# mKaloer/TFServingCache

Hardware: AMD Instinct MI355X
Metric: predict req/sec (whole node) (higher is better)
Workload: dtype bf16; 1 GPU; model=resnet50_v1.5, global_batch=8, seq_len=224, parallelism=ring-sharded serving x1, mode=headline (lru), full=False, batch_per_request=8, threads=10, n_models=1000, model_repo=hardlinked copies of one SavedModel per family (content-dedup applies), provider=disk, pool_size=10, n_cold_loads=1030, transport=real gRPC (native nghttp2 front-end) over TCP loopback, client_channels=1, hipgraph=True

## Files before the change

tfservingcache_amd/engine/csrc/executor.cpp:

```cpp
#include <torch/extension.h>

#include <hip/hip_runtime.h>

#include <c10/hip/HIPStream.h>

#include <cstdint>
#include <stdexcept>
#include <vector>

#include "kernels.h"

namespace tfsc {

enum CallKind : int {
  K_ELT_UNARY = 0,
  K_ELT_BINARY,
  K_BN_ACT,
  K_SOFTMAX,
  K_LAYERNORM,
  K_MEAN_LAST,
  K_MEAN_MID,
  K_POOL,
  K_TRANSPOSE,
  K_GATHER,
  K_PAD_NHWC,
  K_GEMM,
  K_BGEMM,
  K_IM2COL,
  K_CONV,
  K_PAD_LAST,
  K_ATTENTION,
  K_DEPTHWISE,
  K_GEMM_FP8,
  K_QUANT_FP8,
  K_CAST,
  K_ARGMAX_LAST,
  K_SCATTER,
  K_RESIZE,
  K_ZERO_INSERT,
};

struct Call {
  int kind;
  std::vector<intptr_t> ptrs;
  std::vector<int64_t> ints;
  std::vector<float> floats;
};

static void launch_call(const Call& c, hipStream_t s) {
  auto p = [&](int i) { return reinterpret_cast<ushort*>(c.ptrs[i]); };
  auto cp = [&](int i) { return reinterpret_cast<const ushort*>(c.ptrs[i]); };
  const auto& I = c.ints;
  switch (c.kind) {
    case K_ELT_UNARY:
      launch_eltwise_unary(s, cp(0), p(1), I[0], int(I[1]));
      break;
    case K_ELT_BINARY: {
      BcastArgs bc;
      bc.ndim = int(I[2]);
      for (int d = 0; d < MAX_DIMS; ++d) {
        bc.dims[d] = d < bc.ndim ? I[3 + d] : 1;
        bc.sa[d] = d < bc.ndim ? I[3 + bc.ndim + d] : 0;
        bc.sb[d] = d < bc.ndim ? I[3 + 2 * bc.ndim + d] : 0;
      }
      launch_eltwise_binary(s, cp(0), cp(1), p(2), I[0], bc, int(I[1]));
      break;
    }
    case K_BN_ACT:
      launch_bn_act(s, cp(0), cp(1), cp(2), p(3), I[0], I[1], int(I[2]));
      break;
    case K_SOFTMAX:
      launch_softmax(s, cp(0), p(1), I[0], I[1]);
      break;
    case K_LAYERNORM:
      launch_layernorm(s, cp(0), cp(1), cp(2), p(3), I[0], I[1],
                       c.floats[0]);
      break;
    case K_MEAN_LAST:
      launch_reduce_mean_last(s, cp(0), p(1), I[0], I[1]);
      break;
    case K_MEAN_MID:
      launch_reduce_mean_mid(s, cp(0), p(1), I[0], I[1], I[2]);
      break;
    case K_POOL:
      launch_pool(s, cp(0), p(1), I[0] != 0, int(I[1]), int(I[2]),
                  int(I[3]), int(I[4]), int(I[5]), int(I[6]), int(I[7]),
                  int(I[8]), int(I[9]), int(I[10]), int(I[11]), int(I[12]));
      break;
    case K_TRANSPOSE: {
      int ndim = int(I[0]);
      launch_transpose(s, cp(0), p(1), ndim, I.data() + 1,
                       I.data() + 1 + ndim, I[1 + 2 * ndim]);
      break;
    }
    case K_GATHER:
      launch_gather_rows(s, cp(0), reinterpret_cast<const int*>(c.ptrs[1]),
                         p(2), I[0], I[1]);
      break;
    case K_PAD_NHWC:
      launch_pad_nhwc(s, cp(0), p(1), int(I[0]), int(I[1]), int(I[2]),
                      int(I[3]), int(I[4]), int(I[5]), int(I[6]),
                      int(I[7]));
      break;
    case K_GEMM: {
      const ushort* bias = c.ptrs[2] ? cp(2) : nullptr;
      const ushort* res = c.ptrs[3] ? cp(3) : nullptr;
      launch_gemm(s, cp(0), cp(1), bias, res, p(4), I[0], I[1], I[2],
                  int(I[3]), c.floats[0]);
      break;
    }
    case K_BGEMM:
      launch_batched_gemm(s, cp(0), cp(1), p(2), I[0], I[1], I[2], I[3],
                          I[4], I[5], I[6], I[7] != 0, c.floats[0]);
      break;
    case K_IM2COL:
      launch_im2col(s, cp(0), p(1), int(I[0]), int(I[1]), int(I[2]),
                    int(I[3]), int(I[4]), int(I[5]), int(I[6]), int(I[7]),
                    int(I[8]), int(I[9]), int(I[10]), int(I[11]),
                    int(I[12]));
      break;
    case K_CONV: {
      const ushort* res = c.ptrs[3] ? cp(3) : nullptr;
      launch_conv_igemm(s, cp(0), cp(1), cp(2), res, cp(4), p(5),
                        int(I[0]), int(I[1]), int(I[2]), int(I[3]),
                        int(I[4]), int(I[5]), int(I[6]), int(I[7]),
                        int(I[8]), int(I[9]), int(I[10]), int(I[11]),
                        int(I[12]), int(I[13]), int(I[14]));
      break;
    }
    case K_PAD_LAST:
      launch_pad_last(s, cp(0), p(1), I[0], int(I[1]), int(I[2]));
      break;
    case K_ATTENTION: {
      const ushort* abias =
          c.ptrs.size() > 4 && c.ptrs[4] ? cp(4) : nullptr;
      if (abias && I.size() < 7)
        throw std::runtime_error("attention bias needs [sb, sh, sq]");
      launch_attention(s, cp(0), cp(1), cp(2), p(3), int(I[0]), int(I[1]),
                       int(I[2]), int(I[3]), c.floats[0], abias,
                       abias ? I[4] : 0, abias ? I[5] : 0,
                       abias ? I[6] : 0);
      break;
    }
    case K_GEMM_FP8: {
      const ushort* bias8 = c.ptrs[4] ? cp(4) : nullptr;
      const ushort* res8 = c.ptrs[5] ? cp(5) : nullptr;
      launch_gemm_fp8(s, reinterpret_cast<const uint8_t*>(c.ptrs[0]),
                      reinterpret_cast<const float*>(c.ptrs[1]),
                      reinterpret_cast<const uint8_t*>(c.ptrs[2]),
                      reinterpret_cast<const float*>(c.ptrs[3]),
                      bias8, res8, p(6), I[0], I[1], I[2], int(I[3]));
      break;
    }
    case K_QUANT_FP8:
      launch_quant_rowwise(s, cp(0),
                           reinterpret_cast<uint8_t*>(c.ptrs[1]),
                           reinterpret_cast<float*>(c.ptrs[2]),
                           I[0], I[1], I[2]);
      break;
    case K_SCATTER: {
      int nd = int(I[0]);
      launch_scatter(s, cp(0), p(1), nd, I.data() + 1, I.data() + 1 + nd,
                     I[1 + 2 * nd]);
      break;
    }
    case K_CAST:
      launch_cast(s, reinterpret_cast<const void*>(c.ptrs[0]),
                  reinterpret_cast<void*>(c.ptrs[1]), I[0], int(I[1]));
      break;
    case K_ARGMAX_LAST:
      launch_argmax_last(s, cp(0), reinterpret_cast<int*>(c.ptrs[1]),
                         I[0], I[1]);
      break;
    case K_DEPTHWISE:
      launch_depthwise_conv(s, cp(0), cp(1), cp(2), p(3), int(I[0]),
                            int(I[1]), int(I[2]), int(I[3]), int(I[4]),
                            int(I[5]), int(I[6]), int(I[7]), int(I[8]),
                            int(I[9]), int(I[10]), int(I[11]),
                            int(I[12]));
      break;
    case K_RESIZE: {
      if (c.ptrs.size() != 2 || I.size() != 9)
        throw std::runtime_error("resize needs 2 ptrs and 9 ints");
      for (int k = 0; k < 7; ++k)
        if (I[k] < 0 || I[k] > INT32_MAX)
          throw std::runtime_error("resize: int out of range");
      launch_resize_nhwc(s, cp(0), p(1), int(I[0]), int(I[1]), int(I[2]),
                         int(I[3]), int(I[4]), int(I[5]), int(I[6]),
                         I[7] != 0, I[8] != 0);
      break;
    }
    case K_ZERO_INSERT: {
      if (c.ptrs.size() != 2 || I.size() != 6)
        throw std::runtime_error("zero_insert needs 2 ptrs and 6 ints");
      for (int k = 0; k < 6; ++k)
        if (I[k] < 0 || I[k] > INT32_MAX)
          throw std::runtime_error("zero_insert: int out of range");
      launch_zero_insert_nhwc(s, cp(0), p(1), int(I[0]), int(I[1]),
                              int(I[2]), int(I[3]), int(I[4]), int(I[5]));
      break;
    }
    default:
      throw std::runtime_error("unknown call kind " +
                               std::to_string(c.kind));
  }
}

class ExecPlan {
 public:
  explicit ExecPlan(const std::vector<Call>& calls) : calls_(calls) {}

  void run() {
    hipStream_t s = c10::hip::getCurrentHIPStream().stream();
    for (const auto& c : calls_) launch_call(c, s);
    hipError_t e = hipGetLastError();
    if (e != hipSuccess)
      throw std::runtime_error(std::string("kernel launch failed: ") +
                               hipGetErrorString(e));
  }

  void capture() {
    hipStream_t s = c10::hip::getCurrentHIPStream().stream();
    if (graph_exec_) return;
    hipGraph_t graph = nullptr;
    if (hipStreamBeginCapture(s, hipStreamCaptureModeThreadLocal) !=
        hipSuccess)
      throw std::runtime_error("hipStreamBeginCapture failed");
    for (const auto& c : calls_) launch_call(c, s);
    if (hipStreamEndCapture(s, &graph) != hipSuccess)
      throw std::runtime_error("hipStreamEndCapture failed");
    hipGraphExec_t ge = nullptr;
    if (hipGraphInstantiate(&ge, graph, nullptr, nullptr, 0) != hipSuccess) {
      hipGraphDestroy(graph);
      throw std::runtime_error("hipGraphInstantiate failed");
    }
    hipGraphDestroy(graph);
    graph_exec_ = ge;
  }

  bool has_graph() const { return graph_exec_ != nullptr; }

  void run_graph() {
    if (!graph_exec_) {
      run();
      return;
    }
    hipStream_t s = c10::hip::getCurrentHIPStream().stream();
    if (hipGraphLaunch(graph_exec_, s) != hipSuccess)
      throw std::runtime_error("hipGraphLaunch failed");
  }

  ~ExecPlan() {
    if (graph_exec_) hipGraphExecDestroy(graph_exec_);
  }

  void run_on(hipStream_t s) {
    if (graph_exec_) {
      if (hipGraphLaunch(graph_exec_, s) != hipSuccess)
        throw std::runtime_error("hipGraphLaunch failed");
      return;
    }
    for (const auto& c : calls_) launch_call(c, s);
    hipError_t e = hipGetLastError();
    if (e != hipSuccess)
      throw std::runtime_error(std::string("kernel launch failed: ") +
                               hipGetErrorString(e));
  }

  size_t n_calls() const { return calls_.size(); }

 private:
  std::vector<Call> calls_;
  hipGraphExec_t graph_exec_ = nullptr;
};

void fast_run_plan(void* plan, hipStream_t s) {
  reinterpret_cast<ExecPlan*>(plan)->run_on(s);
}

struct PtrDesc {
  uint8_t tag;
  int32_t reg = 0;
  int64_t off = 0;
};

class CallTemplate {
 public:
  std::vector<Call> calls;
  std::vector<std::vector<PtrDesc>> descs;

  ExecPlan* instantiate(uintptr_t ws,
                        const std::vector<uintptr_t>& bases) const {
    std::vector<Call> out = calls;
    for (size_t i = 0; i < out.size(); ++i) {
      auto& ds = descs[i];
      auto& ptrs = out[i].ptrs;
      ptrs.resize(ds.size());
      for (size_t j = 0; j < ds.size(); ++j) {
        const PtrDesc& d = ds[j];
        if (d.tag == 0)
          ptrs[j] = intptr_t(ws) + d.off;
        else if (d.tag == 1)
          ptrs[j] = intptr_t(bases.at(size_t(d.reg))) + d.off;
        else
          ptrs[j] = 0;
      }
    }
    return new ExecPlan(out);
  }
};

}

namespace py = pybind11;

void register_fastpath(py::module_& mod);
void register_frontend(py::module_& mod);
void register_rest_frontend(py::module_& mod);

PYBIND11_MODULE(TORCH_EXTENSION_NAME, mod) {
  using tfsc::Call;
  using tfsc::ExecPlan;

  py::class_<ExecPlan>(mod, "ExecPlan")
      .def(py::init([](py::list calls) {
        std::vector<Call> cs;
        cs.reserve(calls.size());
        for (auto item : calls) {
          py::tuple t = item.cast<py::tuple>();
          Call c;
          c.kind = t[0].cast<int>();
          c.ptrs = t[1].cast<std::vector<intptr_t>>();
          c.ints = t[2].cast<std::vector<int64_t>>();
          c.floats = t[3].cast<std::vector<float>>();
          cs.push_back(std::move(c));
        }
        return new ExecPlan(cs);
      }))
      .def("run", &ExecPlan::run, py::call_guard<py::gil_scoped_release>())
      .def("capture", &ExecPlan::capture,
           py::call_guard<py::gil_scoped_release>())
      .def("run_graph", &ExecPlan::run_graph,
           py::call_guard<py::gil_scoped_release>())
      .def("has_graph", &ExecPlan::has_graph)
      .def("n_calls", &ExecPlan::n_calls)
      .def("ptr", [](ExecPlan& p) {
        return reinterpret_cast<uintptr_t>(&p);
      });

  mod.attr("K_ELT_UNARY") = int(tfsc::K_ELT_UNARY);
  mod.attr("K_ELT_BINARY") = int(tfsc::K_ELT_BINARY);
  mod.attr("K_BN_ACT") = int(tfsc::K_BN_ACT);
  mod.attr("K_SOFTMAX") = int(tfsc::K_SOFTMAX);
  mod.attr("K_LAYERNORM") = int(tfsc::K_LAYERNORM);
  mod.attr("K_MEAN_LAST") = int(tfsc::K_MEAN_LAST);
  mod.attr("K_MEAN_MID") = int(tfsc::K_MEAN_MID);
  mod.attr("K_POOL") = int(tfsc::K_POOL);
  mod.attr("K_TRANSPOSE") = int(tfsc::K_TRANSPOSE);
  mod.attr("K_GATHER") = int(tfsc::K_GATHER);
  mod.attr("K_PAD_NHWC") = int(tfsc::K_PAD_NHWC);
  mod.attr("K_GEMM") = int(tfsc::K_GEMM);
  mod.attr("K_BGEMM") = int(tfsc::K_BGEMM);
  mod.attr("K_IM2COL") = int(tfsc::K_IM2COL);
  mod.attr("K_CONV") = int(tfsc::K_CONV);
  mod.attr("K_PAD_LAST") = int(tfsc::K_PAD_LAST);
  mod.attr("K_ATTENTION") = int(tfsc::K_ATTENTION);
  mod.attr("K_DEPTHWISE") = int(tfsc::K_DEPTHWISE);
  mod.attr("K_GEMM_FP8") = int(tfsc::K_GEMM_FP8);
  mod.attr("K_QUANT_FP8") = int(tfsc::K_QUANT_FP8);
  mod.attr("K_CAST") = int(tfsc::K_CAST);
  mod.attr("K_ARGMAX_LAST") = int(tfsc::K_ARGMAX_LAST);
  mod.attr("K_SCATTER") = int(tfsc::K_SCATTER);
  mod.attr("K_RESIZE") = int(tfsc::K_RESIZE);
  mod.attr("K_ZERO_INSERT") = int(tfsc::K_ZERO_INSERT);

  py::class_<tfsc::CallTemplate>(mod, "CallTemplate")
      .def(py::init([](py::list calls) {
        auto* t = new tfsc::CallTemplate();
        t->calls.reserve(calls.size());
        t->descs.reserve(calls.size());
        for (auto item : calls) {
          py::tuple tu = item.cast<py::tuple>();
          Call c;
          c.kind = tu[0].cast<int>();
          std::vector<tfsc::PtrDesc> ds;
          for (auto dd : tu[1].cast<py::list>()) {
            py::tuple dt = dd.cast<py::tuple>();
            tfsc::PtrDesc d;
            d.tag = uint8_t(dt[0].cast<int>());
            if (d.tag == 0) {
              d.off = dt[1].cast<int64_t>();
            } else if (d.tag == 1) {
              d.reg = dt[1].cast<int32_t>();
              d.off = dt[2].cast<int64_t>();
            }
            ds.push_back(d);
          }
          c.ints = tu[2].cast<std::vector<int64_t>>();
          c.floats = tu[3].cast<std::vector<float>>();
          t->calls.push_back(std::move(c));
          t->descs.push_back(std::move(ds));
        }
        return t;
      }));

  mod.def("instantiate_plan",
          [](const tfsc::CallTemplate& t, uintptr_t ws,
             const std::vector<uintptr_t>& bases) {
            return std::unique_ptr<ExecPlan>(t.instantiate(ws, bases));
          });

  register_fastpath(mod);
  register_frontend(mod);
  register_rest_frontend(mod);

  mod.attr("ELT_ADD") = int(tfsc::ELT_ADD);
  mod.attr("ELT_SUB") = int(tfsc::ELT_SUB);
  mod.attr("ELT_MUL") = int(tfsc::ELT_MUL);
  mod.attr("ELT_DIV") = int(tfsc::ELT_DIV);
  mod.attr("ELT_MAX") = int(tfsc::ELT_MAX);
  mod.attr("ELT_MIN") = int(tfsc::ELT_MIN);
  mod.attr("ELT_SQDIFF") = int(tfsc::ELT_SQDIFF);
  mod.attr("ELT_RELU") = int(tfsc::ELT_RELU);
  mod.attr("ELT_TANH") = int(tfsc::ELT_TANH);
  mod.attr("ELT_SIGMOID") = int(tfsc::ELT_SIGMOID);
  mod.attr("ELT_ERF") = int(tfsc::ELT_ERF);
  mod.attr("ELT_SQRT") = int(tfsc::ELT_SQRT);
  mod.attr("ELT_RSQRT") = int(tfsc::ELT_RSQRT);
  mod.attr("ELT_EXP") = int(tfsc::ELT_EXP);
  mod.attr("ELT_NEG") = int(tfsc::ELT_NEG);
  mod.attr("ELT_SQUARE") = int(tfsc::ELT_SQUARE);
  mod.attr("ELT_GELU") = int(tfsc::ELT_GELU);
  mod.attr("ELT_RELU6") = int(tfsc::ELT_RELU6);

  mod.attr("ACT_NONE") = int(tfsc::ACT_NONE);
  mod.attr("ACT_RELU") = int(tfsc::ACT_RELU);
  mod.attr("ACT_TANH") = int(tfsc::ACT_TANH);
  mod.attr("ACT_SIGMOID") = int(tfsc::ACT_SIGMOID);
  mod.attr("ACT_GELU") = int(tfsc::ACT_GELU);
  mod.attr("ACT_RELU6") = int(tfsc::ACT_RELU6);
}
```

tfservingcache_amd/engine/csrc/ops/attention.hip:

```cpp
#include "../common.h"
#include "../kernels.h"

#include <climits>
#include <stdexcept>

namespace tfsc {

namespace attn {

using bf16x8_t = __attribute__((ext_vector_type(8))) __bf16;
using f32x4_t = __attribute__((ext_vector_type(4))) float;
using ushort2_t = __attribute__((ext_vector_type(2))) ushort;

constexpr int D = 64;
constexpr int QBLK = 64;
constexpr int KVBLK = 64;
constexpr int NW = 4;
constexpr int THREADS = NW * WAVE;

TFSC_DEV int t_off(int row, int chunk) {
  return row * 128 + ((chunk ^ (row & 7)) << 4);
}

TFSC_DEV int p_off(int row, int chunk) {
  return row * 256 + ((chunk ^ (row & 7)) << 4);
}

TFSC_DEV void stage_rows_glds(const ushort* __restrict__ src, int64_t ld,
                              int row0, int row_limit, char* lds_tile,
                              int wave, int lane) {
  int r_in = lane >> 3, chunk = lane & 7;
  #pragma unroll
  for (int i = 0; i < 2; ++i) {
    int row = wave * 16 + i * 8 + r_in;
    int grow = row0 + row;
    grow = grow < row_limit ? grow : row_limit;
    int chunk_src = chunk ^ (row & 7);
    const ushort* gptr = src + (int64_t)grow * ld + chunk_src * 8;
    char* lds_base = lds_tile + (wave * 16 + i * 8) * 128;
    __builtin_amdgcn_global_load_lds(
        reinterpret_cast<const uint32_t*>(gptr),
        reinterpret_cast<uint32_t*>(lds_base), 16, 0, 0);
  }
}

TFSC_DEV void stage_vt(const ushort* __restrict__ src, int64_t ld,
                       int row0, int row_limit, ushort* lds_tile,
                       int wave, int lane) {
  int tid = wave * WAVE + lane;
  #pragma unroll
  for (int pass = 0; pass < 2; ++pass) {
    int idx = pass * THREADS + tid;
    int kv = idx >> 3;
    int dg = idx & 7;
    int gkv = row0 + kv;
    gkv = gkv < row_limit ? gkv : row_limit;
    const ushort* gptr = src + (int64_t)gkv * ld + dg * 8;
    short8_t v = *reinterpret_cast<const short8_t*>(gptr);
    #pragma unroll
    for (int j = 0; j < 8; ++j) {
      int d = dg * 8 + j;
      int byte_off = t_off(d, kv >> 3) + (kv & 7) * 2;
      *reinterpret_cast<ushort*>(
          reinterpret_cast<char*>(lds_tile) + byte_off) = ushort(v[j]);
    }
  }
}

template <int RING, bool HAS_BIAS>
__global__ __launch_bounds__(THREADS)
void attention_kernel(const ushort* __restrict__ Q,
                      const ushort* __restrict__ K,
                      const ushort* __restrict__ V,
                      ushort* __restrict__ O,
                      int B, int S, int H, float scale, int n_qblk,
                      const ushort* __restrict__ bias, int64_t bias_sb,
                      int64_t bias_sh, int bias_sq) {
  __shared__ __attribute__((aligned(16))) char smem[8192 * (2 * RING + 2)];
  auto k_lds = [&](int buf) -> char* { return smem + buf * 8192; };
  auto vt_lds = [&](int buf) -> char* {
    return smem + RING * 8192 + buf * 8192;
  };
  char* q_lds = smem + 2 * RING * 8192;
  char* p_lds = smem + 2 * RING * 8192;

  const int flat = blockIdx.x;
  const int qb = flat % n_qblk;
  const int h = (flat / n_qblk) % H;
  const int b = flat / (n_qblk * H);
  const int64_t ld = (int64_t)H * D;
  const ushort* Qb = Q + (int64_t)b * S * ld + h * D;
  const ushort* Kb = K + (int64_t)b * S * ld + h * D;
  const ushort* Vb = V + (int64_t)b * S * ld + h * D;
  ushort* Ob = O + (int64_t)b * S * ld + h * D;

  const int wave = threadIdx.x / WAVE;
  const int lane = threadIdx.x % WAVE;
  const int frow = lane & 15;
  const int kgrp = lane >> 4;
  const int q0 = qb * QBLK;

  stage_rows_glds(Qb, ld, q0, S - 1, q_lds, wave, lane);
  stage_rows_glds(Kb, ld, 0, S - 1, k_lds(0), wave, lane);
  stage_vt(Vb, ld, 0, S - 1, reinterpret_cast<ushort*>(vt_lds(0)), wave,
           lane);
  stage_rows_glds(Kb, ld, KVBLK, S - 1, k_lds(1), wave, lane);
  stage_vt(Vb, ld, KVBLK, S - 1, reinterpret_cast<ushort*>(vt_lds(1)),
           wave, lane);
  __syncthreads();
  bf16x8_t qf[2];
  #pragma unroll
  for (int ks = 0; ks < 2; ++ks) {
    int row = wave * 16 + frow;
    qf[ks] = *reinterpret_cast<const bf16x8_t*>(
        q_lds + t_off(row, ks * 4 + kgrp));
  }
  __syncthreads();

  float m_run[4], l_run[4];
  f32x4_t o_acc[4] = {};
  #pragma unroll
  for (int r = 0; r < 4; ++r) {
    m_run[r] = HAS_BIAS ? -1.0e38f : -3.0e38f;
    l_run[r] = 0.f;
  }

  const char* bias_bh = nullptr;
  uint32_t bias_roff[4] = {};
  if (HAS_BIAS) {
    bias_bh = reinterpret_cast<const char*>(
        bias + (int64_t)b * bias_sb + (int64_t)h * bias_sh);
    #pragma unroll
    for (int r = 0; r < 4; ++r) {
      int qrow = q0 + wave * 16 + kgrp * 4 + r;
      qrow = qrow < S ? qrow : S - 1;
      bias_roff[r] = uint32_t(qrow) * uint32_t(bias_sq) * 2u;
    }
  }

  const int n_kv = (S + KVBLK - 1) / KVBLK;
  const int n_pair = (n_kv + 1) / 2;

  for (int t = 0; t < n_pair; ++t) {
    if (t > 0) __syncthreads();
    const int base = RING >= 4 ? (t & 1) * 2 : 0;
    const int kv_base = t * 2 * KVBLK;
    ushort2_t bv[4][4] = {};
    if (HAS_BIAS) {
      uint32_t off[8];
      #pragma unroll
      for (int ni = 0; ni < 8; ++ni) {
        int kv_col = kv_base + ni * 16 + frow;
        off[ni] = uint32_t(kv_col < S ? kv_col : S - 1) * 2u;
      }
      if (bias_sq == 0) {
        ushort bk[8];
        #pragma unroll
        for (int ni = 0; ni < 8; ++ni)
          bk[ni] = *reinterpret_cast<const ushort*>(bias_bh + off[ni]);
        #pragma unroll
        for (int ni = 0; ni < 8; ++ni)
          #pragma unroll
          for (int r = 0; r < 4; ++r) bv[ni & 3][r][ni >> 2] = bk[ni];
      } else {
        #pragma unroll
        for (int ni = 0; ni < 8; ++ni)
          #pragma unroll
          for (int r = 0; r < 4; ++r)
            bv[ni & 3][r][ni >> 2] = *reinterpret_cast<const ushort*>(
                bias_bh + (bias_roff[r] + off[ni]));
      }
    }
    if (RING >= 4 && t + 1 < n_pair) {
      const int nb = ((t + 1) & 1) * 2;
      stage_rows_glds(Kb, ld, (2 * t + 2) * KVBLK, S - 1, k_lds(nb),
                      wave, lane);
      stage_vt(Vb, ld, (2 * t + 2) * KVBLK, S - 1,
               reinterpret_cast<ushort*>(vt_lds(nb)), wave, lane);
      stage_rows_glds(Kb, ld, (2 * t + 3) * KVBLK, S - 1, k_lds(nb + 1),
                      wave, lane);
      stage_vt(Vb, ld, (2 * t + 3) * KVBLK, S - 1,
               reinterpret_cast<ushort*>(vt_lds(nb + 1)), wave, lane);
    }

    f32x4_t sc[8] = {};
    #pragma unroll
    for (int half = 0; half < 2; ++half) {
      const char* kt = k_lds(base + half);
      #pragma unroll
      for (int ks = 0; ks < 2; ++ks) {
        #pragma unroll
        for (int ni = 0; ni < 4; ++ni) {
          bf16x8_t kf = *reinterpret_cast<const bf16x8_t*>(
              kt + t_off(ni * 16 + frow, ks * 4 + kgrp));
          sc[half * 4 + ni] = __builtin_amdgcn_mfma_f32_16x16x32_bf16(
              qf[ks], kf, sc[half * 4 + ni], 0, 0, 0);
        }
      }
    }
    #pragma unroll
    for (int ni = 0; ni < 8; ++ni) {
      int kv_col = kv_base + ni * 16 + frow;
      bool valid = kv_col < S;
      #pragma unroll
      for (int r = 0; r < 4; ++r) {
        float v = sc[ni][r] * scale;
        if (HAS_BIAS) v += bf2f(bv[ni & 3][r][ni >> 2]);
        sc[ni][r] = valid ? v : -3.0e38f;
      }
    }

    float pmax[4];
    #pragma unroll
    for (int r = 0; r < 4; ++r) {
      float v = sc[0][r];
      #pragma unroll
      for (int ni = 1; ni < 8; ++ni) v = fmaxf(v, sc[ni][r]);
      #pragma unroll
      for (int off = 8; off > 0; off >>= 1)
        v = fmaxf(v, __shfl_xor(v, off, 16));
      pmax[r] = v;
    }
    float alpha[4];
    #pragma unroll
    for (int r = 0; r < 4; ++r) {
      float m_new = fmaxf(m_run[r], pmax[r]);
      alpha[r] = __expf(m_run[r] - m_new);
      m_run[r] = m_new;
    }
    #pragma unroll
    for (int r = 0; r < 4; ++r) {
      float sum = 0.f;
      #pragma unroll
      for (int ni = 0; ni < 8; ++ni) {
        sc[ni][r] = __expf(sc[ni][r] - m_run[r]);
        sum += sc[ni][r];
      }
      #pragma unroll
      for (int off = 8; off > 0; off >>= 1)
        sum += __shfl_xor(sum, off, 16);
      l_run[r] = l_run[r] * alpha[r] + sum;
    }
    #pragma unroll
    for (int ni = 0; ni < 4; ++ni)
      #pragma unroll
      for (int r = 0; r < 4; ++r)
        o_acc[ni][r] *= alpha[r];

    {
      ushort* pw = reinterpret_cast<ushort*>(p_lds + wave * 4096);
      #pragma unroll
      for (int ni = 0; ni < 8; ++ni) {
        #pragma unroll
        for (int r = 0; r < 4; ++r) {
          int row = kgrp * 4 + r;
          int col = ni * 16 + frow;
          *reinterpret_cast<ushort*>(
              reinterpret_cast<char*>(pw) + p_off(row, col >> 3) +
              (col & 7) * 2) = f2bf(sc[ni][r]);
        }
      }
      const char* pr = reinterpret_cast<const char*>(pw);
      #pragma unroll
      for (int ks = 0; ks < 4; ++ks) {
        bf16x8_t pf = *reinterpret_cast<const bf16x8_t*>(
            pr + p_off(frow, ks * 4 + kgrp));
        const char* vt = vt_lds(base + (ks >> 1));
        int ksub = ks & 1;
        #pragma unroll
        for (int ni = 0; ni < 4; ++ni) {
          bf16x8_t vf = *reinterpret_cast<const bf16x8_t*>(
              vt + t_off(ni * 16 + frow, ksub * 4 + kgrp));
          o_acc[ni] = __builtin_amdgcn_mfma_f32_16x16x32_bf16(
              pf, vf, o_acc[ni], 0, 0, 0);
        }
      }
    }
  }

  #pragma unroll
  for (int r = 0; r < 4; ++r) {
    int row = q0 + wave * 16 + kgrp * 4 + r;
    if (row >= S) continue;
    float inv = l_run[r] > 0.f ? 1.f / l_run[r] : 0.f;
    ushort* orow = Ob + (int64_t)row * ld;
    #pragma unroll
    for (int ni = 0; ni < 4; ++ni)
      orow[ni * 16 + frow] = f2bf(o_acc[ni][r] * inv);
  }
}

}

void launch_attention(hipStream_t s, const ushort* Q, const ushort* K,
                      const ushort* V, ushort* O, int B, int S, int H,
                      int D_, float scale, const ushort* bias,
                      int64_t bias_sb, int64_t bias_sh, int64_t bias_sq) {
  if (D_ != attn::D)
    throw std::runtime_error("fused attention requires head_dim == 64");
  if (bias && (bias_sb < 0 || bias_sh < 0 || bias_sq < 0 ||
               (int64_t)(S - 1) * bias_sq + S > INT32_MAX))
    throw std::runtime_error("fused attention: bad bias strides");
  int n_qblk = (S + attn::QBLK - 1) / attn::QBLK;
  dim3 grid(B * H * n_qblk);
  dim3 block(attn::THREADS);
  const bool small = S <= 2 * attn::KVBLK;
  const int sq = int(bias_sq);
  if (!bias) {
    if (small)
      hipLaunchKernelGGL((attn::attention_kernel<2, false>), grid, block,
                         0, s, Q, K, V, O, B, S, H, scale, n_qblk,
                         nullptr, 0, 0, 0);
    else
      hipLaunchKernelGGL((attn::attention_kernel<4, false>), grid, block,
                         0, s, Q, K, V, O, B, S, H, scale, n_qblk,
                         nullptr, 0, 0, 0);
  } else if (small) {
    hipLaunchKernelGGL((attn::attention_kernel<2, true>), grid, block, 0,
                       s, Q, K, V, O, B, S, H, scale, n_qblk, bias,
                       bias_sb, bias_sh, sq);
  } else {
    hipLaunchKernelGGL((attn::attention_kernel<4, true>), grid, block, 0,
                       s, Q, K, V, O, B, S, H, scale, n_qblk, bias,
                       bias_sb, bias_sh, sq);
  }
}

}
```

tfservingcache_amd/engine/csrc/ops/conv.hip:

```cpp
#include "../common.h"
#include "../kernels.h"

namespace tfsc {

constexpr int TPB = 256;
constexpr int MAX_BLOCKS = 2048;

__global__ void k_im2col_v8(const ushort* __restrict__ x,
                            ushort* __restrict__ y, int N, int H, int W,
                            int C, int R, int S, int sh, int sw, int pt,
                            int pl, int Ho, int Wo, int k_pad) {
  int rsc = R * S * C;
  int c8 = C >> 3;
  int64_t groups_per_m = (int64_t)R * S * c8;
  int64_t n_groups = (int64_t)N * Ho * Wo * groups_per_m;
  int64_t i0 = (int64_t)blockIdx.x * TPB + threadIdx.x;
  int64_t stride = (int64_t)gridDim.x * TPB;
  for (int64_t i = i0; i < n_groups; i += stride) {
    int g = int(i % groups_per_m);
    int64_t mm = i / groups_per_m;
    int c0 = (g % c8) << 3;
    int t = g / c8;
    int ss = t % S, r = t / S;
    int wo = int(mm % Wo);
    int64_t t2 = mm / Wo;
    int ho = int(t2 % Ho);
    int n = int(t2 / Ho);
    int hi = ho * sh + r - pt;
    int wi = wo * sw + ss - pl;
    int k = (r * S + ss) * C + c0;
    ushort* dst = y + mm * k_pad + k;
    if (hi >= 0 && hi < H && wi >= 0 && wi < W) {
      const ushort* src = x + (((int64_t)n * H + hi) * W + wi) * C + c0;
      *reinterpret_cast<uint4*>(dst) =
          *reinterpret_cast<const uint4*>(src);
    } else {
      *reinterpret_cast<uint4*>(dst) = uint4{0, 0, 0, 0};
    }
  }
}

__global__ void k_im2col_padzero(ushort* __restrict__ y, int64_t rows,
                                 int rsc, int k_pad) {
  int tail = k_pad - rsc;
  int64_t n = rows * tail;
  int64_t i0 = (int64_t)blockIdx.x * TPB + threadIdx.x;
  int64_t stride = (int64_t)gridDim.x * TPB;
  for (int64_t i = i0; i < n; i += stride)
    y[(i / tail) * k_pad + rsc + i % tail] = 0;
}

__global__ void k_im2col_row(const ushort* __restrict__ x,
                             ushort* __restrict__ y, int N, int H, int W,
                             int C, int R, int S, int sh, int sw, int pt,
                             int pl, int Ho, int Wo, int k_pad) {
  int sc = S * C;
  int64_t n_rows = (int64_t)N * Ho * Wo * R;
  int64_t i0 = (int64_t)blockIdx.x * TPB + threadIdx.x;
  int64_t stride = (int64_t)gridDim.x * TPB;
  for (int64_t i = i0; i < n_rows; i += stride) {
    int r = int(i % R);
    int64_t mm = i / R;
    int wo = int(mm % Wo);
    int64_t t2 = mm / Wo;
    int ho = int(t2 % Ho);
    int n = int(t2 / Ho);
    int hi = ho * sh + r - pt;
    int wi0 = wo * sw - pl;
    ushort* dst = y + mm * k_pad + r * sc;
    if (hi < 0 || hi >= H) {
      for (int j = 0; j < sc; ++j) dst[j] = 0;
      continue;
    }
    const ushort* src = x + (((int64_t)n * H + hi) * W + wi0) * C;
    for (int ss = 0; ss < S; ++ss) {
      int wi = wi0 + ss;
      bool in = (wi >= 0 && wi < W);
      for (int c = 0; c < C; ++c)
        dst[ss * C + c] = in ? src[ss * C + c] : ushort(0);
    }
  }
}

void launch_im2col(hipStream_t s, const ushort* x, ushort* y,
                   int N, int H, int W, int C, int R, int S,
                   int sh, int sw, int pt, int pl, int Ho, int Wo,
                   int k_pad) {
  int64_t rows = (int64_t)N * Ho * Wo;
  int rsc = R * S * C;
  if (k_pad > rsc) {
    int64_t n = rows * (k_pad - rsc);
    int grid = int(ceil_div(n, (int64_t)TPB));
    if (grid > MAX_BLOCKS) grid = MAX_BLOCKS;
    hipLaunchKernelGGL(k_im2col_padzero, dim3(grid), dim3(TPB), 0, s,
                       y, rows, rsc, k_pad);
  }
  if (C % 8 == 0) {
    int64_t n = rows * R * S * (C / 8);
    int grid = int(ceil_div(n, (int64_t)TPB));
    if (grid > MAX_BLOCKS) grid = MAX_BLOCKS;
    hipLaunchKernelGGL(k_im2col_v8, dim3(grid), dim3(TPB), 0, s, x, y,
                       N, H, W, C, R, S, sh, sw, pt, pl, Ho, Wo, k_pad);
  } else {
    int64_t n = rows * R;
    int grid = int(ceil_div(n, (int64_t)TPB));
    if (grid > MAX_BLOCKS) grid = MAX_BLOCKS;
    hipLaunchKernelGGL(k_im2col_row, dim3(grid), dim3(TPB), 0, s, x, y,
                       N, H, W, C, R, S, sh, sw, pt, pl, Ho, Wo, k_pad);
  }
}

}
```

tfservingcache_amd/engine/csrc/ops/gemm.hip:

```cpp
#include "../common.h"
#include "../kernels.h"

#include <stdexcept>

namespace tfsc {

using bf16x8_t = __attribute__((ext_vector_type(8))) __bf16;
using f32x4_t = __attribute__((ext_vector_type(4))) float;

constexpr int BM = 128, BN = 128, BK = 64;
constexpr int N_WAVES = 4;
constexpr int THREADS = N_WAVES * WAVE;

TFSC_DEV int xcd_swizzle(int bid, int nblocks) {
  constexpr int NXCD = 8;
  if (nblocks < 2 * NXCD) return bid;
  int q = nblocks / NXCD, r = nblocks % NXCD;
  int xcd = bid % NXCD, idx = bid / NXCD;
  return (xcd < r ? xcd * (q + 1) : r * (q + 1) + (xcd - r) * q) + idx;
}

TFSC_DEV int lds_off(int row, int chunk) {
  return row * 128 + ((chunk ^ (row & 7)) << 4);
}

template <int ROWS, int NWAVES>
TFSC_DEV void stage_tile_glds(const ushort* __restrict__ src, int64_t ld,
                              int row_limit, int row0, int k0,
                              char* lds_tile, int wave, int lane) {
  constexpr int ROWS_PER_WAVE = ROWS / NWAVES;
  constexpr int N_GLDS = ROWS_PER_WAVE / 8;
  int r_in = (lane >> 3);
  int chunk = lane & 7;
  #pragma unroll
  for (int i = 0; i < N_GLDS; ++i) {
    int row = wave * ROWS_PER_WAVE + i * 8 + r_in;
    int grow = row0 + row;
    grow = grow < row_limit ? grow : row_limit;
    int chunk_src = chunk ^ (row & 7);
    const ushort* gptr = src + (int64_t)grow * ld + k0 + chunk_src * 8;
    char* lds_base = lds_tile + (wave * ROWS_PER_WAVE + i * 8) * 128;
    __builtin_amdgcn_global_load_lds(
        reinterpret_cast<const uint32_t*>(gptr),
        reinterpret_cast<uint32_t*>(lds_base), 16, 0, 0);
  }
}

template <int ROWS, int NWAVES>
TFSC_DEV void stage_tile_transposed(const ushort* __restrict__ src,
                                    int64_t ld, int k_limit, int n0, int k0,
                                    ushort* lds_tile, int wave, int lane,
                                    int n_limit) {
  constexpr int NG = ROWS / 8;
  constexpr int THREADS_ = NWAVES * WAVE;
  constexpr int PASSES = (ROWS * 64) / (THREADS_ * 8);
  int tid = wave * WAVE + lane;
  #pragma unroll
  for (int pass = 0; pass < PASSES; ++pass) {
    int idx = pass * THREADS_ + tid;
    int k = idx / NG;
    int ng = idx % NG;
    int gk = k0 + k;
    gk = gk < k_limit ? gk : k_limit;
    const ushort* gptr = src + (int64_t)gk * ld + n0 + ng * 8;
    ushort vals[8];
    #pragma unroll
    for (int j = 0; j < 8; ++j) {
      int gn = n0 + ng * 8 + j;
      vals[j] = (gn < n_limit) ? gptr[j] : ushort(0);
    }
    #pragma unroll
    for (int j = 0; j < 8; ++j) {
      int n = ng * 8 + j;
      int byte_off = lds_off(n, k >> 3) + (k & 7) * 2;
      *reinterpret_cast<ushort*>(
          reinterpret_cast<char*>(lds_tile) + byte_off) = vals[j];
    }
  }
}

TFSC_DEV float act_apply(float v, int act) {
  switch (act) {
    case ACT_RELU: return v > 0.f ? v : 0.f;
    case ACT_TANH: return tanhf(v);
    case ACT_SIGMOID: return 1.f / (1.f + __expf(-v));
    case ACT_GELU: return 0.5f * v * (1.f + erff(v * 0.70710678f));
    case ACT_RELU6: return v < 0.f ? 0.f : (v > 6.f ? 6.f : v);
    default: return v;
  }
}

template <bool HAS_BIAS, bool HAS_RES>
TFSC_DEV void epilogue_store(f32x4_t (&acc)[4][4], char* smem,
                             const ushort* __restrict__ bias,
                             const ushort* __restrict__ residual,
                             ushort* __restrict__ Cb,
                             int M, int N, int m0, int n0, int wave,
                             int lane, int wm, int wn, int act,
                             float alpha) {
  __syncthreads();
  ushort* stage = reinterpret_cast<ushort*>(smem + wave * 8192);
  const int col_in = lane & 15;
  const int row_base = (lane >> 4) * 4;
  #pragma unroll
  for (int mi = 0; mi < 4; ++mi) {
    #pragma unroll
    for (int ni = 0; ni < 4; ++ni) {
      int col = ni * 16 + col_in;
      float bv = HAS_BIAS ? bf2f(bias[n0 + wn * 64 + col]) : 0.f;
      #pragma unroll
      for (int r = 0; r < 4; ++r) {
        int row = mi * 16 + row_base + r;
        stage[row * 64 + col] = f2bf(acc[mi][ni][r] * alpha + bv);
      }
    }
  }
  __syncthreads();
  #pragma unroll
  for (int i = 0; i < 8; ++i) {
    int chunk_id = i * 64 + lane;
    int row = chunk_id >> 3;
    int chunk = chunk_id & 7;
    int grow = m0 + wm * 64 + row;
    int gcol0 = n0 + wn * 64 + chunk * 8;
    if (grow >= M) continue;
    bf16x8 v = *reinterpret_cast<const bf16x8*>(stage + row * 64 +
                                                chunk * 8);
    int64_t goff = (int64_t)grow * N + gcol0;
    if (HAS_RES || act != ACT_NONE) {
      bf16x8 rv = {};
      if (HAS_RES && gcol0 + 7 < N)
        rv = *reinterpret_cast<const bf16x8*>(residual + goff);
      #pragma unroll
      for (int j = 0; j < 8; ++j) {
        float x = bf2f((ushort)v[j]);
        if (HAS_RES) {
          if (gcol0 + 7 < N) x += bf2f((ushort)rv[j]);
          else if (gcol0 + j < N) x += bf2f(residual[goff + j]);
        }
        v[j] = (short)f2bf(act_apply(x, act));
      }
    }
    if (gcol0 + 7 < N) {
      *reinterpret_cast<bf16x8*>(Cb + goff) = v;
    } else {
      for (int j = 0; j < 8 && gcol0 + j < N; ++j)
        Cb[goff + j] = (ushort)v[j];
    }
  }
}

template <int WMW, int WNW, bool TRANS_B, bool HAS_BIAS, bool HAS_RES>
__global__ __launch_bounds__(WMW * WNW * WAVE)
void gemm_bf16_kernel(const ushort* __restrict__ A,
                      const ushort* __restrict__ B,
                      const ushort* __restrict__ bias,
                      const ushort* __restrict__ residual,
                      ushort* __restrict__ C,
                      int M, int N, int K, int act, float alpha,
                      int64_t strideA, int64_t strideB, int64_t strideC,
                      int n_tiles_m) {
  constexpr int BM_ = WMW * 64, BN_ = WNW * 64;
  constexpr int NW = WMW * WNW;
  constexpr int A_BYTES = BM_ * BK * 2, B_BYTES = BN_ * BK * 2;
  __shared__ __attribute__((aligned(16))) char smem[2 * (A_BYTES + B_BYTES)];
  auto lds_a = [&](int buf) -> char* {
    return smem + buf * (A_BYTES + B_BYTES); };
  auto lds_b = [&](int buf) -> char* {
    return smem + buf * (A_BYTES + B_BYTES) + A_BYTES; };

  const int bat = blockIdx.y;
  const ushort* Ab = A + bat * strideA;
  const ushort* Bb = B + bat * strideB;
  ushort* Cb = C + bat * strideC;

  const int bid = xcd_swizzle(blockIdx.x, gridDim.x);
  const int tile_m = bid % n_tiles_m;
  const int tile_n = bid / n_tiles_m;
  const int m0 = tile_m * BM_;
  const int n0 = tile_n * BN_;

  const int wave = threadIdx.x / WAVE;
  const int lane = threadIdx.x % WAVE;
  const int wm = wave / WNW, wn = wave % WNW;

  f32x4_t acc[4][4] = {};

  const int n_ktiles = K / BK;

  {
    stage_tile_glds<BM_, NW>(Ab, K, M - 1, m0, 0, lds_a(0), wave, lane);
    if (TRANS_B) {
      stage_tile_glds<BN_, NW>(Bb, K, N - 1, n0, 0, lds_b(0), wave, lane);
    } else {
      stage_tile_transposed<BN_, NW>(
          Bb, N, K - 1, n0, 0, reinterpret_cast<ushort*>(lds_b(0)), wave,
          lane, N);
    }
  }

  int cur = 0;
  for (int kt = 0; kt < n_ktiles; ++kt) {
    __syncthreads();
    if (kt + 1 < n_ktiles) {
      int k0 = (kt + 1) * BK;
      stage_tile_glds<BM_, NW>(Ab, K, M - 1, m0, k0, lds_a(cur ^ 1),
                               wave, lane);
      if (TRANS_B) {
        stage_tile_glds<BN_, NW>(Bb, K, N - 1, n0, k0, lds_b(cur ^ 1),
                                 wave, lane);
      } else {
        stage_tile_transposed<BN_, NW>(
            Bb, N, K - 1, n0, k0,
            reinterpret_cast<ushort*>(lds_b(cur ^ 1)), wave, lane, N);
      }
    }

    const char* at = lds_a(cur);
    const char* bt = lds_b(cur);
    const int frow = lane & 15;
    const int kgrp = lane >> 4;

    #pragma unroll
    for (int ks = 0; ks < 2; ++ks) {
      bf16x8_t a_frag[4], b_frag[4];
      const int chunk = ks * 4 + kgrp;
      #pragma unroll
      for (int mi = 0; mi < 4; ++mi) {
        int row = wm * 64 + mi * 16 + frow;
        a_frag[mi] = *reinterpret_cast<const bf16x8_t*>(
            at + lds_off(row, chunk));
      }
      #pragma unroll
      for (int ni = 0; ni < 4; ++ni) {
        int row = wn * 64 + ni * 16 + frow;
        b_frag[ni] = *reinterpret_cast<const bf16x8_t*>(
            bt + lds_off(row, chunk));
      }
      __builtin_amdgcn_s_setprio(1);
      #pragma unroll
      for (int mi = 0; mi < 4; ++mi)
        #pragma unroll
        for (int ni = 0; ni < 4; ++ni)
          acc[mi][ni] = __builtin_amdgcn_mfma_f32_16x16x32_bf16(
              a_frag[mi], b_frag[ni], acc[mi][ni], 0, 0, 0);
      __builtin_amdgcn_s_setprio(0);
    }
    cur ^= 1;
  }

  epilogue_store<HAS_BIAS, HAS_RES>(acc, smem, bias, residual, Cb, M, N,
                                    m0, n0, wave, lane, wm, wn, act,
                                    alpha);
}

template <int WMW, int WNW, bool TRANS_B>
static void gemm_launch_geom(hipStream_t s, const ushort* A,
                             const ushort* B, const ushort* bias,
                             const ushort* residual, ushort* C,
                             int64_t bat, int64_t M, int64_t N, int64_t K,
                             int act, float alpha, int64_t sA, int64_t sB,
                             int64_t sC) {
  int ntm = int(ceil_div(M, WMW * 64)), ntn = int(ceil_div(N, WNW * 64));
  dim3 grid(ntm * ntn, (unsigned)bat);
  dim3 block(WMW * WNW * WAVE);
  bool hb = bias != nullptr, hr = residual != nullptr;
  auto launch = [&](auto kern) {
    hipLaunchKernelGGL(kern, grid, block, 0, s, A, B, bias, residual, C,
                       (int)M, (int)N, (int)K, act, alpha, sA, sB, sC, ntm);
  };
  if (hb && hr)  launch(gemm_bf16_kernel<WMW, WNW, TRANS_B, true, true>);
  else if (hb)   launch(gemm_bf16_kernel<WMW, WNW, TRANS_B, true, false>);
  else if (hr)   launch(gemm_bf16_kernel<WMW, WNW, TRANS_B, false, true>);
  else           launch(gemm_bf16_kernel<WMW, WNW, TRANS_B, false, false>);
}

template <bool TRANS_B>
static void gemm_dispatch(hipStream_t s, const ushort* A, const ushort* B,
                          const ushort* bias, const ushort* residual,
                          ushort* C, int64_t bat, int64_t M, int64_t N,
                          int64_t K, int act, float alpha, int64_t sA,
                          int64_t sB, int64_t sC) {
  if (K % BK != 0)
    throw std::runtime_error("gemm: K must be a multiple of 64 (got " +
                             std::to_string(K) + ")");
  auto blocks = [&](int bm, int bn) {
    return bat * ceil_div(M, bm) * ceil_div(N, bn);
  };
  if (blocks(128, 128) >= 232) {
    gemm_launch_geom<2, 2, TRANS_B>(s, A, B, bias, residual, C, bat, M, N,
                                    K, act, alpha, sA, sB, sC);
  } else if (blocks(64, 128) >= 232) {
    gemm_launch_geom<1, 2, TRANS_B>(s, A, B, bias, residual, C, bat, M, N,
                                    K, act, alpha, sA, sB, sC);
  } else {
    gemm_launch_geom<1, 1, TRANS_B>(s, A, B, bias, residual, C, bat, M, N,
                                    K, act, alpha, sA, sB, sC);
  }
}

void launch_gemm(hipStream_t s, const ushort* A, const ushort* B,
                 const ushort* bias, const ushort* residual, ushort* C,
                 int64_t M, int64_t N, int64_t K, int act, float alpha) {
  gemm_dispatch<true>(s, A, B, bias, residual, C, 1, M, N, K, act, alpha,
                      0, 0, 0);
}

struct ConvGeom {
  int H, W, C, R, S, sh, sw, pt, pl, Ho, Wo, rsc;
};

TFSC_DEV void stage_tile_conv_a(const ushort* __restrict__ x,
                                const ushort* __restrict__ zeros,
                                const ConvGeom g, int M, int m0, int k0,
                                char* lds_tile, int wave, int lane) {
  int r_in = (lane >> 3);
  int chunk = lane & 7;
  #pragma unroll
  for (int i = 0; i < 4; ++i) {
    int row = wave * 32 + i * 8 + r_in;
    int m = m0 + row;
    m = m < M - 1 ? m : M - 1;
    int chunk_src = chunk ^ (row & 7);
    int k = k0 + chunk_src * 8;
    int wo = m % g.Wo;
    int t = m / g.Wo;
    int ho = t % g.Ho;
    int n = t / g.Ho;
    int c = k % g.C;
    int t2 = k / g.C;
    int s = t2 % g.S;
    int r = t2 / g.S;
    int hi = ho * g.sh + r - g.pt;
    int wi = wo * g.sw + s - g.pl;
    bool ok = (k < g.rsc) & (hi >= 0) & (hi < g.H) & (wi >= 0) & (wi < g.W);
    const ushort* gptr = ok
        ? x + (((int64_t)n * g.H + hi) * g.W + wi) * g.C + c
        : zeros;
    char* lds_base = lds_tile + (wave * 32 + i * 8) * 128;
    __builtin_amdgcn_global_load_lds(
        reinterpret_cast<const uint32_t*>(gptr),
        reinterpret_cast<uint32_t*>(lds_base), 16, 0, 0);
  }
}

template <bool HAS_RES>
__global__ __launch_bounds__(THREADS)
void conv_igemm_kernel(const ushort* __restrict__ x,
                       const ushort* __restrict__ B,
                       const ushort* __restrict__ bias,
                       const ushort* __restrict__ residual,
                       const ushort* __restrict__ zeros,
                       ushort* __restrict__ Cout,
                       int M, int N, int K, int act, ConvGeom g,
                       int n_tiles_m) {
  __shared__ __attribute__((aligned(16))) char smem[4 * BM * BK * 2];
  auto lds_a = [&](int buf) -> char* { return smem + buf * 32768; };
  auto lds_b = [&](int buf) -> char* { return smem + 16384 + buf * 32768; };

  const int bid = xcd_swizzle(blockIdx.x, gridDim.x);
  const int tile_m = bid % n_tiles_m;
  const int tile_n = bid / n_tiles_m;
  const int m0 = tile_m * BM;
  const int n0 = tile_n * BN;
  const int wave = threadIdx.x / WAVE;
  const int lane = threadIdx.x % WAVE;
  const int wm = wave >> 1, wn = wave & 1;

  f32x4_t acc[4][4] = {};
  const int n_ktiles = K / BK;

  stage_tile_conv_a(x, zeros, g, M, m0, 0, lds_a(0), wave, lane);
  stage_tile_glds<128, 4>(B, K, N - 1, n0, 0, lds_b(0), wave, lane);

  int cur = 0;
  for (int kt = 0; kt < n_ktiles; ++kt) {
    __syncthreads();
    if (kt + 1 < n_ktiles) {
      int k0 = (kt + 1) * BK;
      stage_tile_conv_a(x, zeros, g, M, m0, k0, lds_a(cur ^ 1), wave, lane);
      stage_tile_glds<128, 4>(B, K, N - 1, n0, k0, lds_b(cur ^ 1), wave,
                              lane);
    }
    const char* at = lds_a(cur);
    const char* bt = lds_b(cur);
    const int frow = lane & 15;
    const int kgrp = lane >> 4;
    #pragma unroll
    for (int ks = 0; ks < 2; ++ks) {
      bf16x8_t a_frag[4], b_frag[4];
      const int chunk = ks * 4 + kgrp;
      #pragma unroll
      for (int mi = 0; mi < 4; ++mi)
        a_frag[mi] = *reinterpret_cast<const bf16x8_t*>(
            at + lds_off(wm * 64 + mi * 16 + frow, chunk));
      #pragma unroll
      for (int ni = 0; ni < 4; ++ni)
        b_frag[ni] = *reinterpret_cast<const bf16x8_t*>(
            bt + lds_off(wn * 64 + ni * 16 + frow, chunk));
      __builtin_amdgcn_s_setprio(1);
      #pragma unroll
      for (int mi = 0; mi < 4; ++mi)
        #pragma unroll
        for (int ni = 0; ni < 4; ++ni)
          acc[mi][ni] = __builtin_amdgcn_mfma_f32_16x16x32_bf16(
              a_frag[mi], b_frag[ni], acc[mi][ni], 0, 0, 0);
      __builtin_amdgcn_s_setprio(0);
    }
    cur ^= 1;
  }

  epilogue_store<true, HAS_RES>(acc, smem, bias, residual, Cout, M, N,
                                m0, n0, wave, lane, wm, wn, act, 1.0f);
}

void launch_conv_igemm(hipStream_t s, const ushort* x, const ushort* w,
                       const ushort* bias, const ushort* residual,
                       const ushort* zeros, ushort* y,
                       int N_img, int H, int W, int C, int Kc, int R,
                       int S, int sh, int sw, int pt, int pl, int Ho,
                       int Wo, int k_pad, int act) {
  if (C % 8 != 0)
    throw std::runtime_error("conv_igemm requires C % 8 == 0");
  if (k_pad % BK != 0)
    throw std::runtime_error("conv_igemm k_pad must be 64-aligned");
  ConvGeom g{H, W, C, R, S, sh, sw, pt, pl, Ho, Wo, R * S * C};
  int M = N_img * Ho * Wo;
  int ntm = int(ceil_div(M, BM)), ntn = int(ceil_div(Kc, BN));
  dim3 grid(ntm * ntn);
  if (residual)
    hipLaunchKernelGGL((conv_igemm_kernel<true>), grid, dim3(THREADS), 0,
                       s, x, w, bias, residual, zeros, y, M, Kc, k_pad,
                       act, g, ntm);
  else
    hipLaunchKernelGGL((conv_igemm_kernel<false>), grid, dim3(THREADS), 0,
                       s, x, w, bias, nullptr, zeros, y, M, Kc, k_pad,
                       act, g, ntm);
}

void launch_batched_gemm(hipStream_t s, const ushort* A, const ushort* B,
                         ushort* C, int64_t bat, int64_t M, int64_t N,
                         int64_t K, int64_t strideA, int64_t strideB,
                         int64_t strideC, bool trans_b, float alpha) {
  if (trans_b)
    gemm_dispatch<true>(s, A, B, nullptr, nullptr, C, bat, M, N, K,
                        ACT_NONE, alpha, strideA, strideB, strideC);
  else
    gemm_dispatch<false>(s, A, B, nullptr, nullptr, C, bat, M, N, K,
                         ACT_NONE, alpha, strideA, strideB, strideC);
}

}
```

tfservingcache_amd/engine/csrc/ops/gemm_fp8.hip:

```cpp
#include "../common.h"
#include "../kernels.h"

#include <stdexcept>

namespace tfsc {

namespace fp8 {

using i32x4_t = __attribute__((ext_vector_type(4))) int;
using i32x8_t = __attribute__((ext_vector_type(8))) int;
using f32x4_t = __attribute__((ext_vector_type(4))) float;

constexpr int BK = 128;
constexpr int TILE_BYTES_ROW = 128;

TFSC_DEV int xcd_swizzle8(int bid, int nblocks) {
  constexpr int NXCD = 8;
  if (nblocks < 2 * NXCD) return bid;
  int q = nblocks / NXCD, r = nblocks % NXCD;
  int xcd = bid % NXCD, idx = bid / NXCD;
  return (xcd < r ? xcd * (q + 1) : r * (q + 1) + (xcd - r) * q) + idx;
}

TFSC_DEV int lds_off8(int row, int chunk) {
  return row * TILE_BYTES_ROW + ((chunk ^ (row & 7)) << 4);
}

template <int ROWS, int NWAVES>
TFSC_DEV void stage_tile_glds_u8(const uint8_t* __restrict__ src,
                                 int64_t ld, int row_limit, int row0,
                                 int k0, char* lds_tile, int wave,
                                 int lane) {
  constexpr int ROWS_PER_WAVE = ROWS / NWAVES;
  constexpr int N_GLDS = ROWS_PER_WAVE / 8;
  int r_in = (lane >> 3);
  int chunk = lane & 7;
  #pragma unroll
  for (int i = 0; i < N_GLDS; ++i) {
    int row = wave * ROWS_PER_WAVE + i * 8 + r_in;
    int grow = row0 + row;
    grow = grow < row_limit ? grow : row_limit;
    int chunk_src = chunk ^ (row & 7);
    const uint8_t* gptr = src + (int64_t)grow * ld + k0 + chunk_src * 16;
    char* lds_base = lds_tile + (wave * ROWS_PER_WAVE + i * 8) *
                     TILE_BYTES_ROW;
    __builtin_amdgcn_global_load_lds(
        reinterpret_cast<const uint32_t*>(gptr),
        reinterpret_cast<uint32_t*>(lds_base), 16, 0, 0);
  }
}

TFSC_DEV float act8(float v, int act) {
  switch (act) {
    case ACT_RELU: return v > 0.f ? v : 0.f;
    case ACT_TANH: return tanhf(v);
    case ACT_SIGMOID: return 1.f / (1.f + __expf(-v));
    case ACT_GELU: return 0.5f * v * (1.f + erff(v * 0.70710678f));
    case ACT_RELU6: return v < 0.f ? 0.f : (v > 6.f ? 6.f : v);
    default: return v;
  }
}

template <bool HAS_BIAS, bool HAS_RES, int NW>
TFSC_DEV void epilogue_fp8(f32x4_t (&acc)[4][4], char* smem,
                           const float* __restrict__ sa,
                           const float* __restrict__ sb,
                           const ushort* __restrict__ bias,
                           const ushort* __restrict__ residual,
                           ushort* __restrict__ Cb,
                           int M, int N, int m0, int n0, int wave,
                           int lane, int wm, int wn, int act) {
  __syncthreads();
  ushort* stage = reinterpret_cast<ushort*>(smem + wave * 8192);
  const int col_in = lane & 15;
  const int row_base = (lane >> 4) * 4;
  #pragma unroll
  for (int mi = 0; mi < 4; ++mi) {
    #pragma unroll
    for (int ni = 0; ni < 4; ++ni) {
      int col = ni * 16 + col_in;
      int gcol = n0 + wn * 64 + col;
      float bv = HAS_BIAS && gcol < N ? bf2f(bias[gcol]) : 0.f;
      float sbv = gcol < N ? sb[gcol] : 0.f;
      #pragma unroll
      for (int r = 0; r < 4; ++r) {
        int row = mi * 16 + row_base + r;
        int grow = m0 + wm * 64 + row;
        float sav = grow < M ? sa[grow] : 0.f;
        stage[row * 64 + col] = f2bf(acc[mi][ni][r] * sav * sbv + bv);
      }
    }
  }
  __syncthreads();
  #pragma unroll
  for (int i = 0; i < 8; ++i) {
    int chunk_id = i * 64 + lane;
    int row = chunk_id >> 3;
    int chunk = chunk_id & 7;
    int grow = m0 + wm * 64 + row;
    int gcol0 = n0 + wn * 64 + chunk * 8;
    if (grow >= M) continue;
    bf16x8 v = *reinterpret_cast<const bf16x8*>(stage + row * 64 +
                                                chunk * 8);
    int64_t goff = (int64_t)grow * N + gcol0;
    if (HAS_RES || act != ACT_NONE) {
      bf16x8 rv = {};
      if (HAS_RES && gcol0 + 7 < N)
        rv = *reinterpret_cast<const bf16x8*>(residual + goff);
      #pragma unroll
      for (int j = 0; j < 8; ++j) {
        float x = bf2f((ushort)v[j]);
        if (HAS_RES) {
          if (gcol0 + 7 < N) x += bf2f((ushort)rv[j]);
          else if (gcol0 + j < N) x += bf2f(residual[goff + j]);
        }
        v[j] = (short)f2bf(act8(x, act));
      }
    }
    if (gcol0 + 7 < N) {
      *reinterpret_cast<bf16x8*>(Cb + goff) = v;
    } else {
      for (int j = 0; j < 8 && gcol0 + j < N; ++j)
        Cb[goff + j] = (ushort)v[j];
    }
  }
}

template <int WMW, int WNW, bool HAS_BIAS, bool HAS_RES>
__global__ __launch_bounds__(WMW * WNW * WAVE)
void gemm_fp8_kernel(const uint8_t* __restrict__ A,
                     const float* __restrict__ sa,
                     const uint8_t* __restrict__ B,
                     const float* __restrict__ sb,
                     const ushort* __restrict__ bias,
                     const ushort* __restrict__ residual,
                     ushort* __restrict__ C,
                     int M, int N, int K, int act, int n_tiles_m) {
  constexpr int BM_ = WMW * 64, BN_ = WNW * 64;
  constexpr int NW = WMW * WNW;
  constexpr int A_BYTES = BM_ * TILE_BYTES_ROW;
  constexpr int B_BYTES = BN_ * TILE_BYTES_ROW;
  __shared__ __attribute__((aligned(16))) char smem[2 * (A_BYTES + B_BYTES)];
  auto lds_a = [&](int buf) -> char* {
    return smem + buf * (A_BYTES + B_BYTES); };
  auto lds_b = [&](int buf) -> char* {
    return smem + buf * (A_BYTES + B_BYTES) + A_BYTES; };

  const int bid = xcd_swizzle8(blockIdx.x, gridDim.x);
  const int tile_m = bid % n_tiles_m;
  const int tile_n = bid / n_tiles_m;
  const int m0 = tile_m * BM_;
  const int n0 = tile_n * BN_;

  const int wave = threadIdx.x / WAVE;
  const int lane = threadIdx.x % WAVE;
  const int wm = wave / WNW, wn = wave % WNW;

  f32x4_t acc[4][4] = {};
  const int n_ktiles = K / BK;

  stage_tile_glds_u8<BM_, NW>(A, K, M - 1, m0, 0, lds_a(0), wave, lane);
  stage_tile_glds_u8<BN_, NW>(B, K, N - 1, n0, 0, lds_b(0), wave, lane);

  int cur = 0;
  for (int kt = 0; kt < n_ktiles; ++kt) {
    __syncthreads();
    if (kt + 1 < n_ktiles) {
      int k0 = (kt + 1) * BK;
      stage_tile_glds_u8<BM_, NW>(A, K, M - 1, m0, k0, lds_a(cur ^ 1),
                                  wave, lane);
      stage_tile_glds_u8<BN_, NW>(B, K, N - 1, n0, k0, lds_b(cur ^ 1),
                                  wave, lane);
    }
    const char* at = lds_a(cur);
    const char* bt = lds_b(cur);
    const int frow = lane & 15;
    const int kgrp = lane >> 4;

    i32x8_t a_frag[4], b_frag[4];
    #pragma unroll
    for (int mi = 0; mi < 4; ++mi) {
      int row = wm * 64 + mi * 16 + frow;
      i32x4_t lo = *reinterpret_cast<const i32x4_t*>(
          at + lds_off8(row, 2 * kgrp));
      i32x4_t hi = *reinterpret_cast<const i32x4_t*>(
          at + lds_off8(row, 2 * kgrp + 1));
      a_frag[mi] = i32x8_t{lo[0], lo[1], lo[2], lo[3],
                           hi[0], hi[1], hi[2], hi[3]};
    }
    #pragma unroll
    for (int ni = 0; ni < 4; ++ni) {
      int row = wn * 64 + ni * 16 + frow;
      i32x4_t lo = *reinterpret_cast<const i32x4_t*>(
          bt + lds_off8(row, 2 * kgrp));
      i32x4_t hi = *reinterpret_cast<const i32x4_t*>(
          bt + lds_off8(row, 2 * kgrp + 1));
      b_frag[ni] = i32x8_t{lo[0], lo[1], lo[2], lo[3],
                           hi[0], hi[1], hi[2], hi[3]};
    }
    __builtin_amdgcn_s_setprio(1);
    #pragma unroll
    for (int mi = 0; mi < 4; ++mi)
      #pragma unroll
      for (int ni = 0; ni < 4; ++ni)
        acc[mi][ni] = __builtin_amdgcn_mfma_scale_f32_16x16x128_f8f6f4(
            a_frag[mi], b_frag[ni], acc[mi][ni], 0, 0,
            0, 0x7F7F7F7F, 0, 0x7F7F7F7F);
    __builtin_amdgcn_s_setprio(0);
    cur ^= 1;
  }

  epilogue_fp8<HAS_BIAS, HAS_RES, NW>(acc, smem, sa, sb, bias, residual,
                                      C, M, N, m0, n0, wave, lane, wm,
                                      wn, act);
}

TFSC_DEV uint8_t f32_to_e4m3(float f) {
  uint32_t bits = __float_as_uint(f);
  uint8_t sign = uint8_t((bits >> 24) & 0x80);
  float a = fabsf(f);
  if (f != f) return 0x7F;
  if (a >= 448.f) return sign | 0x7E;
  int e = int((bits >> 23) & 0xFF) - 127;
  if (e < -6) {
    int mant = int(a * 512.f + 0.5f);
    if (mant > 7) return sign | 0x08;
    return sign | uint8_t(mant);
  }
  uint32_t mant23 = bits & 0x7FFFFF;
  uint32_t mant3 = (mant23 + 0x80000u) >> 20;
  if (mant3 == 8) {
    mant3 = 0;
    ++e;
    if (e > 8) return sign | 0x7E;
  }
  return sign | uint8_t((e + 7) << 3) | uint8_t(mant3);
}

__global__ __launch_bounds__(256)
void quant_rowwise_kernel(const ushort* __restrict__ x,
                          uint8_t* __restrict__ q,
                          float* __restrict__ scales,
                          int M, int K, int Kp) {
  int wv = threadIdx.x / WAVE;
  int lane = threadIdx.x % WAVE;
  int waves_total = gridDim.x * (256 / WAVE);
  for (int row = blockIdx.x * (256 / WAVE) + wv; row < M;
       row += waves_total) {
    const ushort* xr = x + (int64_t)row * K;
    float amax = 0.f;
    int k4 = K / 4;
    const short4_t* xr4 = reinterpret_cast<const short4_t*>(xr);
    for (int i = lane; i < k4; i += WAVE) {
      short4_t v = xr4[i];
      #pragma unroll
      for (int j = 0; j < 4; ++j)
        amax = fmaxf(amax, fabsf(bf2f((ushort)v[j])));
    }
    for (int i = k4 * 4 + lane; i < K; i += WAVE)
      amax = fmaxf(amax, fabsf(bf2f(xr[i])));
    #pragma unroll
    for (int off = WAVE / 2; off > 0; off >>= 1)
      amax = fmaxf(amax, __shfl_xor(amax, off, WAVE));
    float scale = amax > 0.f ? amax / 448.f : 1.f;
    float inv = 1.f / scale;
    if (lane == 0) scales[row] = scale;
    uint8_t* qr = q + (int64_t)row * Kp;
    for (int i = lane; i < k4; i += WAVE) {
      short4_t v = xr4[i];
      uint32_t outw = 0;
      #pragma unroll
      for (int j = 0; j < 4; ++j)
        outw |= uint32_t(f32_to_e4m3(bf2f((ushort)v[j]) * inv)) << (8 * j);
      reinterpret_cast<uint32_t*>(qr)[i] = outw;
    }
    for (int i = k4 * 4 + lane; i < Kp; i += WAVE)
      qr[i] = i < K ? f32_to_e4m3(bf2f(xr[i]) * inv) : 0;
  }
}

}

void launch_quant_rowwise(hipStream_t s, const ushort* x, uint8_t* q,
                          float* scales, int64_t M, int64_t K,
                          int64_t Kp) {
  int64_t waves_needed = M;
  int blocks = int(ceil_div(waves_needed, (int64_t)(256 / WAVE)));
  if (blocks > 2048) blocks = 2048;
  if (blocks < 1) blocks = 1;
  hipLaunchKernelGGL(fp8::quant_rowwise_kernel, dim3(blocks), dim3(256),
                     0, s, x, q, scales, int(M), int(K), int(Kp));
}

void launch_gemm_fp8(hipStream_t s, const uint8_t* A, const float* sa,
                     const uint8_t* B, const float* sb,
                     const ushort* bias, const ushort* residual,
                     ushort* C, int64_t M, int64_t N, int64_t K,
                     int act) {
  using namespace fp8;
  if (K % BK != 0)
    throw std::runtime_error("gemm_fp8: K must be a multiple of 128");
  auto blocks = [&](int bm, int bn) {
    return ceil_div(M, (int64_t)bm) * ceil_div(N, (int64_t)bn);
  };
  bool hb = bias != nullptr, hr = residual != nullptr;
  auto go = [&](auto kern, int bm, int bn) {
    int ntm = int(ceil_div(M, (int64_t)bm));
    int ntn = int(ceil_div(N, (int64_t)bn));
    dim3 grid(ntm * ntn);
    dim3 block((bm / 64) * (bn / 64) * WAVE);
    hipLaunchKernelGGL(kern, grid, block, 0, s, A, sa, B, sb, bias,
                       residual, C, int(M), int(N), int(K), act, ntm);
  };
  if (blocks(128, 128) >= 232) {
    if (hb && hr)  go(gemm_fp8_kernel<2, 2, true, true>, 128, 128);
    else if (hb)   go(gemm_fp8_kernel<2, 2, true, false>, 128, 128);
    else if (hr)   go(gemm_fp8_kernel<2, 2, false, true>, 128, 128);
    else           go(gemm_fp8_kernel<2, 2, false, false>, 128, 128);
  } else if (blocks(64, 128) >= 232) {
    if (hb && hr)  go(gemm_fp8_kernel<1, 2, true, true>, 64, 128);
    else if (hb)   go(gemm_fp8_kernel<1, 2, true, false>, 64, 128);
    else if (hr)   go(gemm_fp8_kernel<1, 2, false, true>, 64, 128);
    else           go(gemm_fp8_kernel<1, 2, false, false>, 64, 128);
  } else {
    if (hb && hr)  go(gemm_fp8_kernel<1, 1, true, true>, 64, 64);
    else if (hb)   go(gemm_fp8_kernel<1, 1, true, false>, 64, 64);
    else if (hr)   go(gemm_fp8_kernel<1, 1, false, true>, 64, 64);
    else           go(gemm_fp8_kernel<1, 1, false, false>, 64, 64);
  }
}

}
```

tfservingcache_amd/engine/csrc/ops/ops_memory.hip:

```cpp
#include "../common.h"
#include "../kernels.h"

#include <stdexcept>
#include <string>

namespace tfsc {

constexpr int TPB = 256;
constexpr int MAX_BLOCKS = 2048;

static inline int grid_for(int64_t n, int per_thread = 1) {
  int64_t blocks = ceil_div(n, int64_t(TPB) * per_thread);
  return int(blocks < MAX_BLOCKS ? (blocks > 0 ? blocks : 1) : MAX_BLOCKS);
}

TFSC_DEV float apply_unary(float v, int fn) {
  switch (fn) {
    case ELT_RELU: return v > 0.f ? v : 0.f;
    case ELT_TANH: return tanhf(v);
    case ELT_SIGMOID: return 1.f / (1.f + __expf(-v));
    case ELT_ERF: return erff(v);
    case ELT_SQRT: return sqrtf(v);
    case ELT_RSQRT: return rsqrtf(v);
    case ELT_EXP: return __expf(v);
    case ELT_NEG: return -v;
    case ELT_SQUARE: return v * v;
    case ELT_GELU: return 0.5f * v * (1.f + erff(v * 0.70710678f));
    case ELT_RELU6: return v < 0.f ? 0.f : (v > 6.f ? 6.f : v);
    default: return v;
  }
}

TFSC_DEV float apply_binary(float a, float b, int fn) {
  switch (fn) {
    case ELT_ADD: return a + b;
    case ELT_SUB: return a - b;
    case ELT_MUL: return a * b;
    case ELT_DIV: return a / b;
    case ELT_MAX: return fmaxf(a, b);
    case ELT_MIN: return fminf(a, b);
    case ELT_SQDIFF: { float d = a - b; return d * d; }
    default: return a;
  }
}

__global__ void k_unary(const ushort* __restrict__ x, ushort* __restrict__ y,
                        int64_t n, int fn) {
  int64_t i0 = (int64_t)blockIdx.x * TPB + threadIdx.x;
  int64_t stride = (int64_t)gridDim.x * TPB;
  int64_t n4 = n / 4;
  for (int64_t i = i0; i < n4; i += stride) {
    short4_t v = reinterpret_cast<const short4_t*>(x)[i];
    short4_t r;
    #pragma unroll
    for (int j = 0; j < 4; ++j)
      r[j] = (short)f2bf(apply_unary(bf2f((ushort)v[j]), fn));
    reinterpret_cast<short4_t*>(y)[i] = r;
  }
  for (int64_t i = n4 * 4 + i0; i < n; i += stride)
    y[i] = f2bf(apply_unary(bf2f(x[i]), fn));
}

__global__ void k_binary_same(const ushort* __restrict__ a,
                              const ushort* __restrict__ b,
                              ushort* __restrict__ y, int64_t n, int fn) {
  int64_t i0 = (int64_t)blockIdx.x * TPB + threadIdx.x;
  int64_t stride = (int64_t)gridDim.x * TPB;
  int64_t n4 = n / 4;
  for (int64_t i = i0; i < n4; i += stride) {
    short4_t va = reinterpret_cast<const short4_t*>(a)[i];
    short4_t vb = reinterpret_cast<const short4_t*>(b)[i];
    short4_t r;
    #pragma unroll
    for (int j = 0; j < 4; ++j)
      r[j] = (short)f2bf(apply_binary(bf2f((ushort)va[j]),
                                      bf2f((ushort)vb[j]), fn));
    reinterpret_cast<short4_t*>(y)[i] = r;
  }
  for (int64_t i = n4 * 4 + i0; i < n; i += stride)
    y[i] = f2bf(apply_binary(bf2f(a[i]), bf2f(b[i]), fn));
}

__global__ void k_binary_bcast(const ushort* __restrict__ a,
                               const ushort* __restrict__ b,
                               ushort* __restrict__ y, int64_t n,
                               BcastArgs bc, int fn) {
  int64_t i0 = (int64_t)blockIdx.x * TPB + threadIdx.x;
  int64_t stride = (int64_t)gridDim.x * TPB;
  for (int64_t i = i0; i < n; i += stride) {
    int64_t rem = i, ia = 0, ib = 0;
    #pragma unroll
    for (int d = MAX_DIMS - 1; d >= 0; --d) {
      if (d >= bc.ndim) continue;
      int64_t c = rem % bc.dims[d];
      rem /= bc.dims[d];
      ia += c * bc.sa[d];
      ib += c * bc.sb[d];
    }
    y[i] = f2bf(apply_binary(bf2f(a[ia]), bf2f(b[ib]), fn));
  }
}

void launch_eltwise_unary(hipStream_t s, const ushort* x, ushort* y,
                          int64_t n, int fn) {
  hipLaunchKernelGGL(k_unary, dim3(grid_for(n, 4)), dim3(TPB), 0, s,
                     x, y, n, fn);
}

void launch_eltwise_binary(hipStream_t s, const ushort* a, const ushort* b,
                           ushort* y, int64_t n_out, const BcastArgs& bc,
                           int fn) {
  bool same = true;
  for (int d = 0; d < bc.ndim; ++d) {
  }
  if (bc.ndim == 1 && bc.sa[0] == 1 && bc.sb[0] == 1) {
    hipLaunchKernelGGL(k_binary_same, dim3(grid_for(n_out, 4)), dim3(TPB),
                       0, s, a, b, y, n_out, fn);
  } else {
    hipLaunchKernelGGL(k_binary_bcast, dim3(grid_for(n_out)), dim3(TPB),
                       0, s, a, b, y, n_out, bc, fn);
  }
  (void)same;
}

__global__ void k_bn_act(const ushort* __restrict__ x,
                         const ushort* __restrict__ scale,
                         const ushort* __restrict__ shift,
                         ushort* __restrict__ y, int64_t n, int64_t c,
                         int act) {
  int64_t i0 = (int64_t)blockIdx.x * TPB + threadIdx.x;
  int64_t stride = (int64_t)gridDim.x * TPB;
  for (int64_t i = i0; i < n; i += stride) {
    int64_t ch = i % c;
    float v = bf2f(x[i]) * bf2f(scale[ch]) + bf2f(shift[ch]);
    switch (act) {
      case ACT_RELU: v = v > 0.f ? v : 0.f; break;
      case ACT_TANH: v = tanhf(v); break;
      case ACT_SIGMOID: v = 1.f / (1.f + __expf(-v)); break;
      case ACT_GELU: v = 0.5f * v * (1.f + erff(v * 0.70710678f)); break;
      case ACT_RELU6: v = v < 0.f ? 0.f : (v > 6.f ? 6.f : v); break;
    }
    y[i] = f2bf(v);
  }
}

void launch_bn_act(hipStream_t s, const ushort* x, const ushort* scale,
                   const ushort* shift, ushort* y, int64_t rows, int64_t c,
                   int act) {
  int64_t n = rows * c;
  hipLaunchKernelGGL(k_bn_act, dim3(grid_for(n)), dim3(TPB), 0, s,
                     x, scale, shift, y, n, c, act);
}

template <typename Reduce>
TFSC_DEV float block_reduce(float v, Reduce red, float init) {
  __shared__ float smem[TPB / WAVE];
  #pragma unroll
  for (int off = WAVE / 2; off > 0; off >>= 1)
    v = red(v, __shfl_down(v, off, WAVE));
  int wid = threadIdx.x / WAVE;
  if ((threadIdx.x & (WAVE - 1)) == 0) smem[wid] = v;
  __syncthreads();
  v = (threadIdx.x < TPB / WAVE) ? smem[threadIdx.x] : init;
  #pragma unroll
  for (int off = TPB / WAVE / 2; off > 0; off >>= 1)
    v = red(v, __shfl_down(v, off, WAVE));
  v = __shfl(v, 0, WAVE);
  if (threadIdx.x == 0) smem[0] = v;
  __syncthreads();
  v = smem[0];
  __syncthreads();
  return v;
}

struct MaxOp { TFSC_DEV float operator()(float a, float b) const { return fmaxf(a, b); } };
struct SumOp { TFSC_DEV float operator()(float a, float b) const { return a + b; } };

__global__ void k_softmax(const ushort* __restrict__ x,
                          ushort* __restrict__ y, int64_t rows,
                          int64_t cols) {
  for (int64_t row = blockIdx.x; row < rows; row += gridDim.x) {
    const ushort* xr = x + row * cols;
    ushort* yr = y + row * cols;
    float mx = -3.0e38f;
    for (int64_t i = threadIdx.x; i < cols; i += TPB)
      mx = fmaxf(mx, bf2f(xr[i]));
    mx = block_reduce(mx, MaxOp(), -3.0e38f);
    float sum = 0.f;
    for (int64_t i = threadIdx.x; i < cols; i += TPB)
      sum += __expf(bf2f(xr[i]) - mx);
    sum = block_reduce(sum, SumOp(), 0.f);
    float inv = 1.f / sum;
    for (int64_t i = threadIdx.x; i < cols; i += TPB)
      yr[i] = f2bf(__expf(bf2f(xr[i]) - mx) * inv);
  }
}

template <int VPL>
__global__ void k_softmax_wave(const ushort* __restrict__ x,
                               ushort* __restrict__ y, int64_t rows,
                               int cols) {
  int64_t row0 = (int64_t)blockIdx.x * (TPB / WAVE) + threadIdx.x / WAVE;
  int64_t wstride = (int64_t)gridDim.x * (TPB / WAVE);
  int lane = threadIdx.x % WAVE;
  for (int64_t row = row0; row < rows; row += wstride) {
    const ushort* xr = x + row * cols;
    ushort* yr = y + row * cols;
    float v[VPL];
    int n = (cols + WAVE - 1) / WAVE;
    float mx = -3.0e38f;
    #pragma unroll
    for (int j = 0; j < VPL; ++j) {
      int i = j * WAVE + lane;
      v[j] = (j < n && i < cols) ? bf2f(xr[i]) : -3.0e38f;
      mx = fmaxf(mx, v[j]);
    }
    #pragma unroll
    for (int off = WAVE / 2; off > 0; off >>= 1)
      mx = fmaxf(mx, __shfl_xor(mx, off, WAVE));
    float sum = 0.f;
    #pragma unroll
    for (int j = 0; j < VPL; ++j) {
      v[j] = __expf(v[j] - mx);
      sum += v[j];
    }
    #pragma unroll
    for (int off = WAVE / 2; off > 0; off >>= 1)
      sum += __shfl_xor(sum, off, WAVE);
    float inv = 1.f / sum;
    #pragma unroll
    for (int j = 0; j < VPL; ++j) {
      int i = j * WAVE + lane;
      if (j < n && i < cols) yr[i] = f2bf(v[j] * inv);
    }
  }
}

void launch_softmax(hipStream_t s, const ushort* x, ushort* y,
                    int64_t rows, int64_t cols) {
  if (cols <= 512) {
    int64_t wgs = ceil_div(rows, (int64_t)(TPB / WAVE));
    int blocks = int(wgs < MAX_BLOCKS ? (wgs > 0 ? wgs : 1) : MAX_BLOCKS);
    if (cols <= 128)
      hipLaunchKernelGGL(k_softmax_wave<2>, dim3(blocks), dim3(TPB), 0, s,
                         x, y, rows, int(cols));
    else
      hipLaunchKernelGGL(k_softmax_wave<8>, dim3(blocks), dim3(TPB), 0, s,
                         x, y, rows, int(cols));
    return;
  }
  int blocks = int(rows < MAX_BLOCKS ? rows : MAX_BLOCKS);
  hipLaunchKernelGGL(k_softmax, dim3(blocks), dim3(TPB), 0, s,
                     x, y, rows, cols);
}

__global__ void k_layernorm(const ushort* __restrict__ x,
                            const ushort* __restrict__ gamma,
                            const ushort* __restrict__ beta,
                            ushort* __restrict__ y, int64_t rows,
                            int64_t cols, float eps) {
  for (int64_t row = blockIdx.x; row < rows; row += gridDim.x) {
    const ushort* xr = x + row * cols;
    ushort* yr = y + row * cols;
    float sum = 0.f, sq = 0.f;
    for (int64_t i = threadIdx.x; i < cols; i += TPB) {
      float v = bf2f(xr[i]);
      sum += v;
      sq += v * v;
    }
    sum = block_reduce(sum, SumOp(), 0.f);
    sq = block_reduce(sq, SumOp(), 0.f);
    float mean = sum / cols;
    float var = sq / cols - mean * mean;
    float rstd = rsqrtf(var > 0.f ? var + eps : eps);
    for (int64_t i = threadIdx.x; i < cols; i += TPB) {
      float v = (bf2f(xr[i]) - mean) * rstd;
      yr[i] = f2bf(v * bf2f(gamma[i]) + bf2f(beta[i]));
    }
  }
}

void launch_layernorm(hipStream_t s, const ushort* x, const ushort* gamma,
                      const ushort* beta, ushort* y, int64_t rows,
                      int64_t cols, float eps) {
  int blocks = int(rows < MAX_BLOCKS ? rows : MAX_BLOCKS);
  hipLaunchKernelGGL(k_layernorm, dim3(blocks), dim3(TPB), 0, s,
                     x, gamma, beta, y, rows, cols, eps);
}

__global__ void k_mean_last(const ushort* __restrict__ x,
                            ushort* __restrict__ y, int64_t rows,
                            int64_t cols) {
  for (int64_t row = blockIdx.x; row < rows; row += gridDim.x) {
    const ushort* xr = x + row * cols;
    float sum = 0.f;
    for (int64_t i = threadIdx.x; i < cols; i += TPB)
      sum += bf2f(xr[i]);
    sum = block_reduce(sum, SumOp(), 0.f);
    if (threadIdx.x == 0) y[row] = f2bf(sum / cols);
  }
}

void launch_reduce_mean_last(hipStream_t s, const ushort* x, ushort* y,
                             int64_t rows, int64_t cols) {
  int blocks = int(rows < MAX_BLOCKS ? rows : MAX_BLOCKS);
  hipLaunchKernelGGL(k_mean_last, dim3(blocks), dim3(TPB), 0, s,
                     x, y, rows, cols);
}

__global__ void k_mean_mid(const ushort* __restrict__ x,
                           ushort* __restrict__ y, int64_t d0, int64_t d1,
                           int64_t d2) {
  int64_t n = d0 * d2;
  int64_t i0 = (int64_t)blockIdx.x * TPB + threadIdx.x;
  int64_t stride = (int64_t)gridDim.x * TPB;
  for (int64_t i = i0; i < n; i += stride) {
    int64_t o = i / d2, c = i % d2;
    const ushort* xp = x + o * d1 * d2 + c;
    float sum = 0.f;
    for (int64_t j = 0; j < d1; ++j) sum += bf2f(xp[j * d2]);
    y[i] = f2bf(sum / d1);
  }
}

void launch_reduce_mean_mid(hipStream_t s, const ushort* x, ushort* y,
                            int64_t d0, int64_t d1, int64_t d2) {
  hipLaunchKernelGGL(k_mean_mid, dim3(grid_for(d0 * d2)), dim3(TPB), 0, s,
                     x, y, d0, d1, d2);
}

void launch_global_mean(hipStream_t s, const ushort* x, ushort* y,
                        int64_t n, int64_t hw, int64_t c) {
  launch_reduce_mean_mid(s, x, y, n, hw, c);
}

__global__ void k_pool(const ushort* __restrict__ x, ushort* __restrict__ y,
                       bool is_max, int N, int H, int W, int C, int Ho,
                       int Wo, int kh, int kw, int sh, int sw, int pt,
                       int pl) {
  int64_t n_out = (int64_t)N * Ho * Wo * C;
  int64_t i0 = (int64_t)blockIdx.x * TPB + threadIdx.x;
  int64_t stride = (int64_t)gridDim.x * TPB;
  for (int64_t i = i0; i < n_out; i += stride) {
    int c = int(i % C);
    int64_t t = i / C;
    int wo = int(t % Wo); t /= Wo;
    int ho = int(t % Ho); int n = int(t / Ho);
    float acc = is_max ? -3.0e38f : 0.f;
    int count = 0;
    for (int r = 0; r < kh; ++r) {
      int hi = ho * sh + r - pt;
      if (hi < 0 || hi >= H) continue;
      for (int q = 0; q < kw; ++q) {
        int wi = wo * sw + q - pl;
        if (wi < 0 || wi >= W) continue;
        float v = bf2f(x[(((int64_t)n * H + hi) * W + wi) * C + c]);
        if (is_max) acc = fmaxf(acc, v);
        else acc += v;
        ++count;
      }
    }
    y[i] = f2bf(is_max ? acc : (count ? acc / count : 0.f));
  }
}

__global__ void k_pool_v8(const ushort* __restrict__ x,
                          ushort* __restrict__ y, bool is_max, int N,
                          int H, int W, int C, int Ho, int Wo, int kh,
                          int kw, int sh, int sw, int pt, int pl) {
  int c8 = C >> 3;
  int64_t n_grp = (int64_t)N * Ho * Wo * c8;
  int64_t i0 = (int64_t)blockIdx.x * TPB + threadIdx.x;
  int64_t stride = (int64_t)gridDim.x * TPB;
  for (int64_t i = i0; i < n_grp; i += stride) {
    int g = int(i % c8);
    int64_t t = i / c8;
    int wo = int(t % Wo); t /= Wo;
    int ho = int(t % Ho); int n = int(t / Ho);
    float acc[8];
    #pragma unroll
    for (int j = 0; j < 8; ++j) acc[j] = is_max ? -3.0e38f : 0.f;
    int count = 0;
    for (int r = 0; r < kh; ++r) {
      int hi = ho * sh + r - pt;
      if (hi < 0 || hi >= H) continue;
      for (int q = 0; q < kw; ++q) {
        int wi = wo * sw + q - pl;
        if (wi < 0 || wi >= W) continue;
        short4_t lo = *reinterpret_cast<const short4_t*>(
            x + (((int64_t)n * H + hi) * W + wi) * C + g * 8);
        short4_t hi4 = *reinterpret_cast<const short4_t*>(
            x + (((int64_t)n * H + hi) * W + wi) * C + g * 8 + 4);
        #pragma unroll
        for (int j = 0; j < 4; ++j) {
          float a = bf2f((ushort)lo[j]);
          float b = bf2f((ushort)hi4[j]);
          if (is_max) {
            acc[j] = fmaxf(acc[j], a);
            acc[j + 4] = fmaxf(acc[j + 4], b);
          } else {
            acc[j] += a;
            acc[j + 4] += b;
          }
        }
        ++count;
      }
    }
    short4_t out_lo, out_hi;
    #pragma unroll
    for (int j = 0; j < 4; ++j) {
      float a = is_max ? acc[j] : (count ? acc[j] / count : 0.f);
      float b = is_max ? acc[j + 4] : (count ? acc[j + 4] / count : 0.f);
      out_lo[j] = (short)f2bf(a);
      out_hi[j] = (short)f2bf(b);
    }
    ushort* dst = y + i * 8;
    *reinterpret_cast<short4_t*>(dst) = out_lo;
    *reinterpret_cast<short4_t*>(dst + 4) = out_hi;
  }
}

void launch_pool(hipStream_t s, const ushort* x, ushort* y, bool is_max,
                 int N, int H, int W, int C, int Ho, int Wo, int kh, int kw,
                 int sh, int sw, int pt, int pl) {
  if (C % 8 == 0) {
    int64_t n_grp = (int64_t)N * Ho * Wo * (C / 8);
    hipLaunchKernelGGL(k_pool_v8, dim3(grid_for(n_grp)), dim3(TPB), 0, s,
                       x, y, is_max, N, H, W, C, Ho, Wo, kh, kw, sh, sw,
                       pt, pl);
    return;
  }
  int64_t n_out = (int64_t)N * Ho * Wo * C;
  hipLaunchKernelGGL(k_pool, dim3(grid_for(n_out)), dim3(TPB), 0, s,
                     x, y, is_max, N, H, W, C, Ho, Wo, kh, kw, sh, sw,
                     pt, pl);
}

struct TransArgs {
  int ndim;
  int64_t out_dims[MAX_DIMS];
  int64_t in_strides[MAX_DIMS];
};

__global__ void k_transpose(const ushort* __restrict__ x,
                            ushort* __restrict__ y, TransArgs ta,
                            int64_t n) {
  int64_t i0 = (int64_t)blockIdx.x * TPB + threadIdx.x;
  int64_t stride = (int64_t)gridDim.x * TPB;
  for (int64_t i = i0; i < n; i += stride) {
    int64_t rem = i, src = 0;
    #pragma unroll
    for (int d = MAX_DIMS - 1; d >= 0; --d) {
      if (d >= ta.ndim) continue;
      int64_t c = rem % ta.out_dims[d];
      rem /= ta.out_dims[d];
      src += c * ta.in_strides[d];
    }
    y[i] = x[src];
  }
}

__global__ void k_transpose_v8(const ushort* __restrict__ x,
                               ushort* __restrict__ y, TransArgs ta,
                               int64_t n_grp, int last) {
  int grp_per_row = last >> 3;
  int64_t i0 = (int64_t)blockIdx.x * TPB + threadIdx.x;
  int64_t stride = (int64_t)gridDim.x * TPB;
  for (int64_t i = i0; i < n_grp; i += stride) {
    int g = int(i % grp_per_row);
    int64_t rem = i / grp_per_row;
    int64_t src = 0;
    #pragma unroll
    for (int d = MAX_DIMS - 1; d >= 0; --d) {
      if (d >= ta.ndim - 1) continue;
      int64_t c = rem % ta.out_dims[d];
      rem /= ta.out_dims[d];
      src += c * ta.in_strides[d];
    }
    *reinterpret_cast<uint4*>(y + i * 8) =
        *reinterpret_cast<const uint4*>(x + src + g * 8);
  }
}

void launch_transpose(hipStream_t s, const ushort* x, ushort* y, int ndim,
                      const int64_t* out_dims, const int64_t* in_strides,
                      int64_t n_out) {
  TransArgs ta;
  ta.ndim = ndim;
  for (int d = 0; d < MAX_DIMS; ++d) {
    ta.out_dims[d] = d < ndim ? out_dims[d] : 1;
    ta.in_strides[d] = d < ndim ? in_strides[d] : 0;
  }
  int last = ndim > 0 ? int(out_dims[ndim - 1]) : 0;
  if (ndim >= 2 && in_strides[ndim - 1] == 1 && last % 8 == 0) {
    int64_t n_grp = n_out / 8;
    hipLaunchKernelGGL(k_transpose_v8, dim3(grid_for(n_grp)), dim3(TPB),
                       0, s, x, y, ta, n_grp, last);
    return;
  }
  hipLaunchKernelGGL(k_transpose, dim3(grid_for(n_out)), dim3(TPB), 0, s,
                     x, y, ta, n_out);
}

__global__ void k_gather_rows(const ushort* __restrict__ table,
                              const int* __restrict__ idx,
                              ushort* __restrict__ y, int64_t n_idx,
                              int64_t row) {
  int64_t n = n_idx * row;
  int64_t i0 = (int64_t)blockIdx.x * TPB + threadIdx.x;
  int64_t stride = (int64_t)gridDim.x * TPB;
  for (int64_t i = i0; i < n; i += stride) {
    int64_t r = i / row, c = i % row;
    y[i] = table[(int64_t)idx[r] * row + c];
  }
}

void launch_gather_rows(hipStream_t s, const ushort* table, const int* idx,
                        ushort* y, int64_t n_idx, int64_t row_elems) {
  hipLaunchKernelGGL(k_gather_rows, dim3(grid_for(n_idx * row_elems)),
                     dim3(TPB), 0, s, table, idx, y, n_idx, row_elems);
}

__global__ void k_f32_to_bf16(const float* __restrict__ x,
                              ushort* __restrict__ y, int64_t n) {
  int64_t i0 = (int64_t)blockIdx.x * TPB + threadIdx.x;
  int64_t stride = (int64_t)gridDim.x * TPB;
  int64_t n4 = n / 4;
  for (int64_t i = i0; i < n4; i += stride) {
    float4 v = reinterpret_cast<const float4*>(x)[i];
    short4_t r;
    r[0] = (short)f2bf(v.x); r[1] = (short)f2bf(v.y);
    r[2] = (short)f2bf(v.z); r[3] = (short)f2bf(v.w);
    reinterpret_cast<short4_t*>(y)[i] = r;
  }
  for (int64_t i = n4 * 4 + i0; i < n; i += stride)
    y[i] = f2bf(x[i]);
}

__global__ void k_bf16_to_f32(const ushort* __restrict__ x,
                              float* __restrict__ y, int64_t n) {
  int64_t i0 = (int64_t)blockIdx.x * TPB + threadIdx.x;
  int64_t stride = (int64_t)gridDim.x * TPB;
  int64_t n4 = n / 4;
  for (int64_t i = i0; i < n4; i += stride) {
    short4_t v = reinterpret_cast<const short4_t*>(x)[i];
    float4 r;
    r.x = bf2f((ushort)v[0]); r.y = bf2f((ushort)v[1]);
    r.z = bf2f((ushort)v[2]); r.w = bf2f((ushort)v[3]);
    reinterpret_cast<float4*>(y)[i] = r;
  }
  for (int64_t i = n4 * 4 + i0; i < n; i += stride)
    y[i] = bf2f(x[i]);
}

void launch_f32_to_bf16(hipStream_t s, const float* x, ushort* y,
                        int64_t n) {
  hipLaunchKernelGGL(k_f32_to_bf16, dim3(grid_for(n, 4)), dim3(TPB), 0, s,
                     x, y, n);
}

void launch_bf16_to_f32(hipStream_t s, const ushort* x, float* y,
                        int64_t n) {
  hipLaunchKernelGGL(k_bf16_to_f32, dim3(grid_for(n, 4)), dim3(TPB), 0, s,
                     x, y, n);
}

__global__ void k_pad_last(const ushort* __restrict__ x,
                           ushort* __restrict__ y, int64_t rows, int c_in,
                           int c_out) {
  int64_t n = rows * c_out;
  int64_t i0 = (int64_t)blockIdx.x * TPB + threadIdx.x;
  int64_t stride = (int64_t)gridDim.x * TPB;
  for (int64_t i = i0; i < n; i += stride) {
    int c = int(i % c_out);
    int64_t r = i / c_out;
    y[i] = c < c_in ? x[r * c_in + c] : ushort(0);
  }
}

void launch_pad_last(hipStream_t s, const ushort* x, ushort* y,
                     int64_t rows, int c_in, int c_out) {
  hipLaunchKernelGGL(k_pad_last, dim3(grid_for(rows * c_out)), dim3(TPB),
                     0, s, x, y, rows, c_in, c_out);
}

__global__ void k_pad_nhwc(const ushort* __restrict__ x,
                           ushort* __restrict__ y, int N, int H, int W,
                           int C, int pt, int pl, int Ho, int Wo) {
  int64_t n_out = (int64_t)N * Ho * Wo * C;
  int64_t i0 = (int64_t)blockIdx.x * TPB + threadIdx.x;
  int64_t stride = (int64_t)gridDim.x * TPB;
  for (int64_t i = i0; i < n_out; i += stride) {
    int c = int(i % C);
    int64_t t = i / C;
    int wo = int(t % Wo); t /= Wo;
    int ho = int(t % Ho); int n = int(t / Ho);
    int hi = ho - pt, wi = wo - pl;
    ushort v = 0;
    if (hi >= 0 && hi < H && wi >= 0 && wi < W)
      v = x[(((int64_t)n * H + hi) * W + wi) * C + c];
    y[i] = v;
  }
}

void launch_pad_nhwc(hipStream_t s, const ushort* x, ushort* y,
                     int N, int H, int W, int C, int pt, int pb, int pl,
                     int pr) {
  int Ho = H + pt + pb, Wo = W + pl + pr;
  int64_t n_out = (int64_t)N * Ho * Wo * C;
  hipLaunchKernelGGL(k_pad_nhwc, dim3(grid_for(n_out)), dim3(TPB), 0, s,
                     x, y, N, H, W, C, pt, pl, Ho, Wo);
}

TFSC_DEV float dw_act(float v, int act) {
  switch (act) {
    case ACT_RELU: return v > 0.f ? v : 0.f;
    case ACT_TANH: return tanhf(v);
    case ACT_SIGMOID: return 1.f / (1.f + __expf(-v));
    case ACT_GELU: return 0.5f * v * (1.f + erff(v * 0.70710678f));
    case ACT_RELU6: return v < 0.f ? 0.f : (v > 6.f ? 6.f : v);
    default: return v;
  }
}

__global__ void k_depthwise_v4(const ushort* __restrict__ x,
                               const ushort* __restrict__ w,
                               const ushort* __restrict__ bias,
                               ushort* __restrict__ y,
                               int N, int H, int W, int C, int R, int S,
                               int sh, int sw, int pt, int pl,
                               int Ho, int Wo, int act) {
  int c4 = C / 4;
  int64_t total = (int64_t)N * Ho * Wo * c4;
  int64_t i0 = (int64_t)blockIdx.x * TPB + threadIdx.x;
  int64_t stride = (int64_t)gridDim.x * TPB;
  for (int64_t i = i0; i < total; i += stride) {
    int64_t t = i;
    int cv = int(t % c4); t /= c4;
    int wo = int(t % Wo); t /= Wo;
    int ho = int(t % Ho); int n = int(t / Ho);
    int c = cv * 4;
    float acc[4];
    short4_t bv = reinterpret_cast<const short4_t*>(bias)[cv];
    #pragma unroll
    for (int j = 0; j < 4; ++j) acc[j] = bf2f((ushort)bv[j]);
    int hi0 = ho * sh - pt, wi0 = wo * sw - pl;
    for (int r = 0; r < R; ++r) {
      int hi = hi0 + r;
      if (hi < 0 || hi >= H) continue;
      for (int sx = 0; sx < S; ++sx) {
        int wi = wi0 + sx;
        if (wi < 0 || wi >= W) continue;
        short4_t xv = reinterpret_cast<const short4_t*>(
            x + ((((int64_t)n * H + hi) * W + wi) * C))[cv];
        short4_t wv = reinterpret_cast<const short4_t*>(
            w + ((r * S + sx) * C))[cv];
        #pragma unroll
        for (int j = 0; j < 4; ++j)
          acc[j] += bf2f((ushort)xv[j]) * bf2f((ushort)wv[j]);
      }
    }
    short4_t out;
    #pragma unroll
    for (int j = 0; j < 4; ++j)
      out[j] = (short)f2bf(dw_act(acc[j], act));
    reinterpret_cast<short4_t*>(
        y + ((((int64_t)n * Ho + ho) * Wo + wo) * C))[cv] = out;
  }
}

__global__ void k_depthwise_scalar(const ushort* __restrict__ x,
                                   const ushort* __restrict__ w,
                                   const ushort* __restrict__ bias,
                                   ushort* __restrict__ y,
                                   int N, int H, int W, int C, int R, int S,
                                   int sh, int sw, int pt, int pl,
                                   int Ho, int Wo, int act) {
  int64_t total = (int64_t)N * Ho * Wo * C;
  int64_t i0 = (int64_t)blockIdx.x * TPB + threadIdx.x;
  int64_t stride = (int64_t)gridDim.x * TPB;
  for (int64_t i = i0; i < total; i += stride) {
    int64_t t = i;
    int c = int(t % C); t /= C;
    int wo = int(t % Wo); t /= Wo;
    int ho = int(t % Ho); int n = int(t / Ho);
    float acc = bf2f(bias[c]);
    int hi0 = ho * sh - pt, wi0 = wo * sw - pl;
    for (int r = 0; r < R; ++r) {
      int hi = hi0 + r;
      if (hi < 0 || hi >= H) continue;
      for (int sx = 0; sx < S; ++sx) {
        int wi = wi0 + sx;
        if (wi < 0 || wi >= W) continue;
        acc += bf2f(x[(((int64_t)n * H + hi) * W + wi) * C + c]) *
               bf2f(w[(r * S + sx) * C + c]);
      }
    }
    y[i] = f2bf(dw_act(acc, act));
  }
}

void launch_depthwise_conv(hipStream_t s, const ushort* x, const ushort* w,
                           const ushort* bias, ushort* y,
                           int N, int H, int W, int C, int R, int S,
                           int sh, int sw, int pt, int pl, int Ho, int Wo,
                           int act) {
  if (C % 4 == 0) {
    int64_t total = (int64_t)N * Ho * Wo * (C / 4);
    hipLaunchKernelGGL(k_depthwise_v4, dim3(grid_for(total)), dim3(TPB),
                       0, s, x, w, bias, y, N, H, W, C, R, S, sh, sw,
                       pt, pl, Ho, Wo, act);
  } else {
    int64_t total = (int64_t)N * Ho * Wo * C;
    hipLaunchKernelGGL(k_depthwise_scalar, dim3(grid_for(total)),
                       dim3(TPB), 0, s, x, w, bias, y, N, H, W, C, R, S,
                       sh, sw, pt, pl, Ho, Wo, act);
  }
}

__global__ void k_scatter(const ushort* __restrict__ x,
                          ushort* __restrict__ y, TransArgs ta,
                          int64_t n) {
  int64_t i0 = (int64_t)blockIdx.x * TPB + threadIdx.x;
  int64_t stride = (int64_t)gridDim.x * TPB;
  for (int64_t i = i0; i < n; i += stride) {
    int64_t rem = i, dst = 0;
    #pragma unroll
    for (int d = MAX_DIMS - 1; d >= 0; --d) {
      if (d >= ta.ndim) continue;
      int64_t c = rem % ta.out_dims[d];
      rem /= ta.out_dims[d];
      dst += c * ta.in_strides[d];
    }
    y[dst] = x[i];
  }
}

void launch_scatter(hipStream_t s, const ushort* x, ushort* y, int ndim,
                    const int64_t* in_dims, const int64_t* out_strides,
                    int64_t n_in) {
  TransArgs ta;
  ta.ndim = ndim;
  for (int d = 0; d < MAX_DIMS; ++d) {
    ta.out_dims[d] = d < ndim ? in_dims[d] : 1;
    ta.in_strides[d] = d < ndim ? out_strides[d] : 0;
  }
  hipLaunchKernelGGL(k_scatter, dim3(grid_for(n_in)), dim3(TPB), 0, s,
                     x, y, ta, n_in);
}

__global__ void k_cast_i2f(const int* __restrict__ x,
                           ushort* __restrict__ y, int64_t n) {
  int64_t i0 = (int64_t)blockIdx.x * TPB + threadIdx.x;
  int64_t stride = (int64_t)gridDim.x * TPB;
  for (int64_t i = i0; i < n; i += stride)
    y[i] = f2bf(float(x[i]));
}

__global__ void k_cast_f2i(const ushort* __restrict__ x,
                           int* __restrict__ y, int64_t n) {
  int64_t i0 = (int64_t)blockIdx.x * TPB + threadIdx.x;
  int64_t stride = (int64_t)gridDim.x * TPB;
  for (int64_t i = i0; i < n; i += stride)
    y[i] = int(bf2f(x[i]));
}

void launch_cast(hipStream_t s, const void* x, void* y, int64_t n,
                 int mode) {
  if (mode == 0)
    hipLaunchKernelGGL(k_cast_i2f, dim3(grid_for(n)), dim3(TPB), 0, s,
                       reinterpret_cast<const int*>(x),
                       reinterpret_cast<ushort*>(y), n);
  else
    hipLaunchKernelGGL(k_cast_f2i, dim3(grid_for(n)), dim3(TPB), 0, s,
                       reinterpret_cast<const ushort*>(x),
                       reinterpret_cast<int*>(y), n);
}

__global__ __launch_bounds__(256)
void k_argmax_last(const ushort* __restrict__ x, int* __restrict__ y,
                   int64_t rows, int64_t cols) {
  int wv = threadIdx.x / WAVE;
  int lane = threadIdx.x % WAVE;
  int64_t waves_total = (int64_t)gridDim.x * (256 / WAVE);
  for (int64_t row = (int64_t)blockIdx.x * (256 / WAVE) + wv;
       row < rows; row += waves_total) {
    const ushort* xr = x + row * cols;
    float best = -3.0e38f;
    int besti = 0x7FFFFFFF;
    for (int64_t i = lane; i < cols; i += WAVE) {
      float v = bf2f(xr[i]);
      if (v > best || (v == best && int(i) < besti)) {
        best = v;
        besti = int(i);
      }
    }
    #pragma unroll
    for (int off = WAVE / 2; off > 0; off >>= 1) {
      float ov = __shfl_xor(best, off, WAVE);
      int oi = __shfl_xor(besti, off, WAVE);
      if (ov > best || (ov == best && oi < besti)) {
        best = ov;
        besti = oi;
      }
    }
    if (lane == 0) y[row] = besti;
  }
}

void launch_argmax_last(hipStream_t s, const ushort* x, int* y,
                        int64_t rows, int64_t cols) {
  int64_t waves = rows;
  int blocks = int(ceil_div(waves, (int64_t)(256 / WAVE)));
  if (blocks > 2048) blocks = 2048;
  if (blocks < 1) blocks = 1;
  hipLaunchKernelGGL(k_argmax_last, dim3(blocks), dim3(256), 0, s, x, y,
                     rows, cols);
}

struct ResizeGeom {
  int N, H, W, C, Ho, Wo;
  int align, half;
  float hscale, wscale;
};

TFSC_DEV int resize_nearest_idx(int d, float scale, int n_in, int align,
                                int half) {
  float src = half ? __fmul_rn(float(d) + 0.5f, scale)
                   : __fmul_rn(float(d), scale);
  int i = int(align ? roundf(src) : floorf(src));
  return min(max(i, 0), n_in - 1);
}

TFSC_DEV void resize_bilinear_coord(int d, float scale, int n_in, int half,
                                    int& lo, int& hi, float& lerp) {
  float src = half ? __fsub_rn(__fmul_rn(float(d) + 0.5f, scale), 0.5f)
                   : __fmul_rn(float(d), scale);
  float fl = floorf(src);
  lo = min(max(int(fl), 0), n_in - 1);
  hi = min(max(int(ceilf(src)), 0), n_in - 1);
  lerp = src - fl;
}

TFSC_DEV float resize_lerp2(float tl, float tr, float bl, float br,
                            float lx, float ly) {
  float top = tl + (tr - tl) * lx;
  float bot = bl + (br - bl) * lx;
  return top + (bot - top) * ly;
}

TFSC_DEV float bf_lo(uint32_t u) { return __uint_as_float(u << 16); }
TFSC_DEV float bf_hi(uint32_t u) { return __uint_as_float(u & 0xffff0000u); }

TFSC_DEV uint32_t resize_lerp_pair(uint32_t tl, uint32_t tr, uint32_t bl,
                                   uint32_t br, float lx, float ly) {
  return f2bf2(
      resize_lerp2(bf_lo(tl), bf_lo(tr), bf_lo(bl), bf_lo(br), lx, ly),
      resize_lerp2(bf_hi(tl), bf_hi(tr), bf_hi(bl), bf_hi(br), lx, ly));
}

template <bool BILINEAR>
__global__ void k_resize_v8(const ushort* __restrict__ x,
                            ushort* __restrict__ y, ResizeGeom g) {
  int c8 = g.C >> 3;
  int64_t n_grp = (int64_t)g.N * g.Ho * g.Wo * c8;
  int64_t i0 = (int64_t)blockIdx.x * TPB + threadIdx.x;
  int64_t stride = (int64_t)gridDim.x * TPB;
  for (int64_t i = i0; i < n_grp; i += stride) {
    int grp = int(i % c8);
    int64_t t = i / c8;
    int wo = int(t % g.Wo); t /= g.Wo;
    int ho = int(t % g.Ho); int n = int(t / g.Ho);
    const ushort* img = x + (int64_t)n * g.H * g.W * g.C + grp * 8;
    auto px = [&](int hi, int wi) {
      return *reinterpret_cast<const uint4*>(
          img + ((int64_t)hi * g.W + wi) * g.C);
    };
    uint4 out;
    if (BILINEAR) {
      int y0, y1, x0, x1;
      float ly, lx;
      resize_bilinear_coord(ho, g.hscale, g.H, g.half, y0, y1, ly);
      resize_bilinear_coord(wo, g.wscale, g.W, g.half, x0, x1, lx);
      uint4 tl = px(y0, x0), tr = px(y0, x1);
      uint4 bl = px(y1, x0), br = px(y1, x1);
      out.x = resize_lerp_pair(tl.x, tr.x, bl.x, br.x, lx, ly);
      out.y = resize_lerp_pair(tl.y, tr.y, bl.y, br.y, lx, ly);
      out.z = resize_lerp_pair(tl.z, tr.z, bl.z, br.z, lx, ly);
      out.w = resize_lerp_pair(tl.w, tr.w, bl.w, br.w, lx, ly);
    } else {
      out = px(resize_nearest_idx(ho, g.hscale, g.H, g.align, g.half),
               resize_nearest_idx(wo, g.wscale, g.W, g.align, g.half));
    }
    *reinterpret_cast<uint4*>(y + i * 8) = out;
  }
}

template <bool BILINEAR>
__global__ void k_resize(const ushort* __restrict__ x,
                         ushort* __restrict__ y, ResizeGeom g) {
  int64_t n_out = (int64_t)g.N * g.Ho * g.Wo * g.C;
  int64_t i0 = (int64_t)blockIdx.x * TPB + threadIdx.x;
  int64_t stride = (int64_t)gridDim.x * TPB;
  for (int64_t i = i0; i < n_out; i += stride) {
    int c = int(i % g.C);
    int64_t t = i / g.C;
    int wo = int(t % g.Wo); t /= g.Wo;
    int ho = int(t % g.Ho); int n = int(t / g.Ho);
    const ushort* img = x + (int64_t)n * g.H * g.W * g.C + c;
    auto px = [&](int hi, int wi) {
      return img[((int64_t)hi * g.W + wi) * g.C];
    };
    if (BILINEAR) {
      int y0, y1, x0, x1;
      float ly, lx;
      resize_bilinear_coord(ho, g.hscale, g.H, g.half, y0, y1, ly);
      resize_bilinear_coord(wo, g.wscale, g.W, g.half, x0, x1, lx);
      y[i] = f2bf(resize_lerp2(bf2f(px(y0, x0)), bf2f(px(y0, x1)),
                               bf2f(px(y1, x0)), bf2f(px(y1, x1)),
                               lx, ly));
    } else {
      y[i] = px(resize_nearest_idx(ho, g.hscale, g.H, g.align, g.half),
                resize_nearest_idx(wo, g.wscale, g.W, g.align, g.half));
    }
  }
}

static inline bool aligned16(const void* a, const void* b) {
  return ((reinterpret_cast<uintptr_t>(a) | reinterpret_cast<uintptr_t>(b)) &
          15u) == 0;
}

static inline float resize_scale(int n_in, int n_out, bool align_corners) {
  return (align_corners && n_out > 1)
             ? float(n_in - 1) / float(n_out - 1)
             : float(n_in) / float(n_out);
}

void launch_resize_nhwc(hipStream_t s, const ushort* x, ushort* y, int N,
                        int H, int W, int C, int Ho, int Wo, int mode,
                        bool align_corners, bool half_pixel_centers) {
  if (N <= 0 || H <= 0 || W <= 0 || C <= 0 || Ho <= 0 || Wo <= 0)
    throw std::runtime_error("resize: every dimension must be positive");
  if (mode != 0 && mode != 1)
    throw std::runtime_error("resize: mode must be 0 (nearest) or 1 "
                             "(bilinear), got " + std::to_string(mode));
  if (align_corners && half_pixel_centers)
    throw std::runtime_error("resize: align_corners and "
                             "half_pixel_centers are mutually exclusive");
  ResizeGeom g{N, H, W, C, Ho, Wo, align_corners ? 1 : 0,
               half_pixel_centers ? 1 : 0,
               resize_scale(H, Ho, align_corners),
               resize_scale(W, Wo, align_corners)};
  if (C % 8 == 0 && aligned16(x, y)) {
    int64_t n_grp = (int64_t)N * Ho * Wo * (C / 8);
    if (mode == 1)
      hipLaunchKernelGGL(k_resize_v8<true>, dim3(grid_for(n_grp)),
                         dim3(TPB), 0, s, x, y, g);
    else
      hipLaunchKernelGGL(k_resize_v8<false>, dim3(grid_for(n_grp)),
                         dim3(TPB), 0, s, x, y, g);
    return;
  }
  int64_t n_out = (int64_t)N * Ho * Wo * C;
  if (mode == 1)
    hipLaunchKernelGGL(k_resize<true>, dim3(grid_for(n_out)), dim3(TPB), 0,
                       s, x, y, g);
  else
    hipLaunchKernelGGL(k_resize<false>, dim3(grid_for(n_out)), dim3(TPB), 0,
                       s, x, y, g);
}

__global__ void k_zero_insert_v8(const ushort* __restrict__ x,
                                 ushort* __restrict__ y, int N, int h,
                                 int w, int C, int sh, int sw, int Ho,
                                 int Wo) {
  int c8 = C >> 3;
  int64_t n_grp = (int64_t)N * Ho * Wo * c8;
  int64_t i0 = (int64_t)blockIdx.x * TPB + threadIdx.x;
  int64_t stride = (int64_t)gridDim.x * TPB;
  for (int64_t i = i0; i < n_grp; i += stride) {
    int grp = int(i % c8);
    int64_t t = i / c8;
    int wo = int(t % Wo); t /= Wo;
    int ho = int(t % Ho); int n = int(t / Ho);
    uint4 v = uint4{0, 0, 0, 0};
    if (ho % sh == 0 && wo % sw == 0)
      v = *reinterpret_cast<const uint4*>(
          x + (((int64_t)n * h + ho / sh) * w + wo / sw) * C + grp * 8);
    *reinterpret_cast<uint4*>(y + i * 8) = v;
  }
}

__global__ void k_zero_insert(const ushort* __restrict__ x,
                              ushort* __restrict__ y, int N, int h, int w,
                              int C, int sh, int sw, int Ho, int Wo) {
  int64_t n_out = (int64_t)N * Ho * Wo * C;
  int64_t i0 = (int64_t)blockIdx.x * TPB + threadIdx.x;
  int64_t stride = (int64_t)gridDim.x * TPB;
  for (int64_t i = i0; i < n_out; i += stride) {
    int c = int(i % C);
    int64_t t = i / C;
    int wo = int(t % Wo); t /= Wo;
    int ho = int(t % Ho); int n = int(t / Ho);
    ushort v = 0;
    if (ho % sh == 0 && wo % sw == 0)
      v = x[(((int64_t)n * h + ho / sh) * w + wo / sw) * C + c];
    y[i] = v;
  }
}

void launch_zero_insert_nhwc(hipStream_t s, const ushort* x, ushort* y,
                             int N, int h, int w, int C, int sh, int sw) {
  if (N <= 0 || h <= 0 || w <= 0 || C <= 0 || sh <= 0 || sw <= 0)
    throw std::runtime_error(
        "zero_insert: every dimension and stride must be positive");
  int64_t Ho64 = (int64_t)(h - 1) * sh + 1, Wo64 = (int64_t)(w - 1) * sw + 1;
  if (Ho64 > INT32_MAX || Wo64 > INT32_MAX)
    throw std::runtime_error("zero_insert: output image too large");
  int Ho = int(Ho64), Wo = int(Wo64);
  if (C % 8 == 0 && aligned16(x, y)) {
    int64_t n_grp = (int64_t)N * Ho * Wo * (C / 8);
    hipLaunchKernelGGL(k_zero_insert_v8, dim3(grid_for(n_grp)), dim3(TPB),
                       0, s, x, y, N, h, w, C, sh, sw, Ho, Wo);
    return;
  }
  int64_t n_out = (int64_t)N * Ho * Wo * C;
  hipLaunchKernelGGL(k_zero_insert, dim3(grid_for(n_out)), dim3(TPB), 0, s,
                     x, y, N, h, w, C, sh, sw, Ho, Wo);
}

}
```

Measured before the change: 312.9 req/s.

## Build HIP graphs directly from recorded kernel launches instead of stream capture

Adds a launch recorder: every kernel launch goes through a `tfsc_launch` wrapper that, when a thread-local recorder is active, stores the function pointer, launch geometry and packed arguments instead of launching. A new `ExecPlan::build_graph` replays the plan into this recorder and assembles a linear hipGraph with `hipGraphAddKernelNode`, avoiding stream-capture overhead on cold model loads. It also adds build timing and global counters for built versus fallback-captured graphs. The Python side is not changed here, so the existing capture path stays in use unless a caller invokes `build_graph`. Every launch now pays a thread-local pointer check.

```diff
diff --git a/tfservingcache_amd/engine/csrc/executor.cpp b/tfservingcache_amd/engine/csrc/executor.cpp
--- a/tfservingcache_amd/engine/csrc/executor.cpp
+++ b/tfservingcache_amd/engine/csrc/executor.cpp
@@ -4,11 +4,14 @@
 
 #include <c10/hip/HIPStream.h>
 
+#include <atomic>
+#include <chrono>
 #include <cstdint>
 #include <stdexcept>
 #include <vector>
 
 #include "kernels.h"
+#include "launch.h"
 
 namespace tfsc {
 
@@ -206,6 +209,12 @@
   }
 }
 
+struct GraphBuildStats {
+  std::atomic<uint64_t> built{0};
+  std::atomic<uint64_t> fallback_capture{0};
+};
+static GraphBuildStats g_graph_stats;
+
 class ExecPlan {
  public:
   explicit ExecPlan(const std::vector<Call>& calls) : calls_(calls) {}
@@ -219,9 +228,20 @@
                                hipGetErrorString(e));
   }
 
+  void build_graph() {
+    if (graph_exec_) return;
+    try {
+      build_graph_impl();
+    } catch (...) {
+      build_failed_ = true;
+      throw;
+    }
+  }
+
   void capture() {
     hipStream_t s = c10::hip::getCurrentHIPStream().stream();
     if (graph_exec_) return;
+    if (build_failed_) ++g_graph_stats.fallback_capture;
     hipGraph_t graph = nullptr;
     if (hipStreamBeginCapture(s, hipStreamCaptureModeThreadLocal) !=
         hipSuccess)
@@ -268,10 +288,73 @@
   }
 
   size_t n_calls() const { return calls_.size(); }
+  size_t n_nodes() const { return descs_.size(); }
+
+  double record_ms() const { return record_ms_; }
+  double graph_ms() const { return graph_ms_; }
 
  private:
+  void build_graph_impl() {
+    using clk = std::chrono::steady_clock;
+    auto ms = [](clk::time_point a, clk::time_point b) {
+      return std::chrono::duration<double, std::milli>(b - a).count();
+    };
+    auto fail = [](const char* what, hipError_t e) {
+      return std::runtime_error(std::string(what) + " failed: " +
+                                hipGetErrorString(e));
+    };
+    auto t0 = clk::now();
+    LaunchRecorder rec;
+    {
+      LaunchRecorder::Scope scope(&rec);
+      for (const auto& c : calls_) launch_call(c, nullptr);
+    }
+    auto t1 = clk::now();
+    std::vector<KernelNodeDesc>& descs = rec.nodes;
+    std::vector<std::vector<void*>> argvs(descs.size());
+
+    hipGraph_t graph = nullptr;
+    hipError_t e = hipGraphCreate(&graph, 0);
+    if (e != hipSuccess) throw fail("hipGraphCreate", e);
+    hipGraphNode_t prev = nullptr;
+    for (size_t i = 0; i < descs.size(); ++i) {
+      KernelNodeDesc& d = descs[i];
+      argvs[i] = d.param_ptrs();
+      hipKernelNodeParams p{};
+      p.func = const_cast<void*>(d.func);
+      p.gridDim = d.grid;
+      p.blockDim = d.block;
+      p.sharedMemBytes = d.shmem;
+      p.kernelParams = argvs[i].data();
+      p.extra = nullptr;
+      hipGraphNode_t node = nullptr;
+      e = hipGraphAddKernelNode(&node, graph, prev ? &prev : nullptr,
+                                prev ? 1 : 0, &p);
+      if (e != hipSuccess) {
+        hipGraphDestroy(graph);
+        throw fail("hipGraphAddKernelNode", e);
+      }
+      prev = node;
+    }
+    hipGraphExec_t ge = nullptr;
+    e = hipGraphInstantiate(&ge, graph, nullptr, nullptr, 0);
+    hipGraphDestroy(graph);
+    if (e != hipSuccess) throw fail("hipGraphInstantiate", e);
+    descs_ = std::move(rec.nodes);
+    argvs_ = std::move(argvs);
+    graph_exec_ = ge;
+    record_ms_ = ms(t0, t1);
+    graph_ms_ = ms(t1, clk::now());
+    ++g_graph_stats.built;
+  }
+
   std::vector<Call> calls_;
   hipGraphExec_t graph_exec_ = nullptr;
+  std::vector<KernelNodeDesc> descs_;
+  std::vector<std::vector<void*>> argvs_;
+  bool build_failed_ = false;
+  double record_ms_ = 0.0;
+  double graph_ms_ = 0.0;
 };
 
 void fast_run_plan(void* plan, hipStream_t s) {
@@ -342,8 +425,17 @@
            py::call_guard<py::gil_scoped_release>())
       .def("run_graph", &ExecPlan::run_graph,
            py::call_guard<py::gil_scoped_release>())
+      .def("build_graph", &ExecPlan::build_graph,
+           py::call_guard<py::gil_scoped_release>())
       .def("has_graph", &ExecPlan::has_graph)
       .def("n_calls", &ExecPlan::n_calls)
+      .def("n_nodes", &ExecPlan::n_nodes)
+      .def("build_timing", [](ExecPlan& p) {
+        py::dict d;
+        d["record_ms"] = p.record_ms();
+        d["graph_ms"] = p.graph_ms();
+        return d;
+      })
       .def("ptr", [](ExecPlan& p) {
         return reinterpret_cast<uintptr_t>(&p);
       });
@@ -410,6 +502,13 @@
             return std::unique_ptr<ExecPlan>(t.instantiate(ws, bases));
           });
 
+  mod.def("graph_build_stats", []() {
+    py::dict d;
+    d["built"] = tfsc::g_graph_stats.built.load();
+    d["fallback_capture"] = tfsc::g_graph_stats.fallback_capture.load();
+    return d;
+  });
+
   register_fastpath(mod);
   register_frontend(mod);
   register_rest_frontend(mod);
diff --git a/tfservingcache_amd/engine/csrc/launch.h b/tfservingcache_amd/engine/csrc/launch.h
--- /dev/null
+++ b/tfservingcache_amd/engine/csrc/launch.h
@@ -0,0 +1,114 @@
+#pragma once
+
+#include <hip/hip_runtime.h>
+
+#include <cstddef>
+#include <cstdint>
+#include <cstring>
+#include <type_traits>
+#include <utility>
+#include <vector>
+
+namespace tfsc {
+
+struct KernelNodeDesc {
+  static constexpr size_t kBlobAlign = 16;
+  struct alignas(kBlobAlign) Chunk {
+    unsigned char bytes[kBlobAlign];
+  };
+
+  const void* func = nullptr;
+  dim3 grid{1, 1, 1};
+  dim3 block{1, 1, 1};
+  unsigned shmem = 0;
+  std::vector<Chunk> blob;
+  std::vector<uint32_t> offsets;
+  size_t blob_bytes = 0;
+
+  size_t n_args() const { return offsets.size(); }
+  unsigned char* data() {
+    return blob.empty() ? nullptr : blob[0].bytes;
+  }
+  const unsigned char* data() const {
+    return blob.empty() ? nullptr : blob[0].bytes;
+  }
+  void* arg(size_t i) { return data() + offsets[i]; }
+  const void* arg(size_t i) const { return data() + offsets[i]; }
+
+  std::vector<void*> param_ptrs() {
+    std::vector<void*> out(offsets.size());
+    for (size_t i = 0; i < offsets.size(); ++i) out[i] = arg(i);
+    return out;
+  }
+
+  template <typename T>
+  void push(const T& v) {
+    static_assert(std::is_trivially_copyable<T>::value,
+                  "kernel arguments must be trivially copyable");
+    static_assert(alignof(T) <= kBlobAlign,
+                  "kernel argument over-aligned for the blob");
+    size_t off = (blob_bytes + alignof(T) - 1) / alignof(T) * alignof(T);
+    size_t end = off + sizeof(T);
+    size_t chunks = (end + kBlobAlign - 1) / kBlobAlign;
+    if (chunks > blob.size()) blob.resize(chunks);
+    std::memcpy(data() + off, &v, sizeof(T));
+    offsets.push_back(uint32_t(off));
+    blob_bytes = end;
+  }
+};
+
+class LaunchRecorder {
+ public:
+  std::vector<KernelNodeDesc> nodes;
+
+  static LaunchRecorder*& current() {
+    static thread_local LaunchRecorder* cur = nullptr;
+    return cur;
+  }
+
+  class Scope {
+   public:
+    explicit Scope(LaunchRecorder* r) : prev_(current()) { current() = r; }
+    ~Scope() { current() = prev_; }
+    Scope(const Scope&) = delete;
+    Scope& operator=(const Scope&) = delete;
+
+   private:
+    LaunchRecorder* prev_;
+  };
+};
+
+namespace detail {
+template <typename... KArgs>
+struct RecordTyped {
+  static void put(LaunchRecorder* r, const void* func, dim3 grid,
+                  dim3 block, unsigned shmem, KArgs... vals) {
+    r->nodes.emplace_back();
+    KernelNodeDesc& d = r->nodes.back();
+    d.func = func;
+    d.grid = grid;
+    d.block = block;
+    d.shmem = shmem;
+    d.offsets.reserve(sizeof...(KArgs));
+    (d.push<typename std::remove_cv<KArgs>::type>(vals), ...);
+  }
+};
+}
+
+template <typename... KArgs, typename... Args>
+inline void tfsc_launch(void (*kernel)(KArgs...), dim3 grid, dim3 block,
+                        unsigned shmem, hipStream_t stream,
+                        Args&&... args) {
+  static_assert(sizeof...(KArgs) == sizeof...(Args),
+                "argument count does not match the kernel's parameters");
+  if (LaunchRecorder* r = LaunchRecorder::current()) {
+    detail::RecordTyped<KArgs...>::put(
+        r, reinterpret_cast<const void*>(kernel), grid, block, shmem,
+        std::forward<Args>(args)...);
+    return;
+  }
+  hipLaunchKernelGGL(kernel, grid, block, shmem, stream,
+                     std::forward<Args>(args)...);
+}
+
+}
diff --git a/tfservingcache_amd/engine/csrc/ops/attention.hip b/tfservingcache_amd/engine/csrc/ops/attention.hip
--- a/tfservingcache_amd/engine/csrc/ops/attention.hip
+++ b/tfservingcache_amd/engine/csrc/ops/attention.hip
@@ -1,5 +1,6 @@
 #include "../common.h"
 #include "../kernels.h"
+#include "../launch.h"
 
 #include <climits>
 #include <stdexcept>
@@ -308,22 +309,22 @@
   const int sq = int(bias_sq);
   if (!bias) {
     if (small)
-      hipLaunchKernelGGL((attn::attention_kernel<2, false>), grid, block,
-                         0, s, Q, K, V, O, B, S, H, scale, n_qblk,
-                         nullptr, 0, 0, 0);
+      tfsc_launch((attn::attention_kernel<2, false>), grid, block,
+                  0, s, Q, K, V, O, B, S, H, scale, n_qblk,
+                  nullptr, 0, 0, 0);
     else
-      hipLaunchKernelGGL((attn::attention_kernel<4, false>), grid, block,
-                         0, s, Q, K, V, O, B, S, H, scale, n_qblk,
-                         nullptr, 0, 0, 0);
+      tfsc_launch((attn::attention_kernel<4, false>), grid, block,
+                  0, s, Q, K, V, O, B, S, H, scale, n_qblk,
+                  nullptr, 0, 0, 0);
   } else if (small) {
-    hipLaunchKernelGGL((attn::attention_kernel<2, true>), grid, block, 0,
-                       s, Q, K, V, O, B, S, H, scale, n_qblk, bias,
-                       bias_sb, bias_sh, sq);
+    tfsc_launch((attn::attention_kernel<2, true>), grid, block, 0,
+                s, Q, K, V, O, B, S, H, scale, n_qblk, bias,
+                bias_sb, bias_sh, sq);
   } else {
-    hipLaunchKernelGGL((attn::attention_kernel<4, true>), grid, block, 0,
-                       s, Q, K, V, O, B, S, H, scale, n_qblk, bias,
-                       bias_sb, bias_sh, sq);
-  }
-}
-
-}
+    tfsc_launch((attn::attention_kernel<4, true>), grid, block, 0,
+                s, Q, K, V, O, B, S, H, scale, n_qblk, bias,
+                bias_sb, bias_sh, sq);
+  }
+}
+
+}
diff --git a/tfservingcache_amd/engine/csrc/ops/conv.hip b/tfservingcache_amd/engine/csrc/ops/conv.hip
--- a/tfservingcache_amd/engine/csrc/ops/conv.hip
+++ b/tfservingcache_amd/engine/csrc/ops/conv.hip
@@ -1,5 +1,6 @@
 #include "../common.h"
 #include "../kernels.h"
+#include "../launch.h"
 
 namespace tfsc {
 
@@ -92,21 +93,21 @@
     int64_t n = rows * (k_pad - rsc);
     int grid = int(ceil_div(n, (int64_t)TPB));
     if (grid > MAX_BLOCKS) grid = MAX_BLOCKS;
-    hipLaunchKernelGGL(k_im2col_padzero, dim3(grid), dim3(TPB), 0, s,
-                       y, rows, rsc, k_pad);
+    tfsc_launch(k_im2col_padzero, dim3(grid), dim3(TPB), 0, s,
+                y, rows, rsc, k_pad);
   }
   if (C % 8 == 0) {
     int64_t n = rows * R * S * (C / 8);
     int grid = int(ceil_div(n, (int64_t)TPB));
     if (grid > MAX_BLOCKS) grid = MAX_BLOCKS;
-    hipLaunchKernelGGL(k_im2col_v8, dim3(grid), dim3(TPB), 0, s, x, y,
-                       N, H, W, C, R, S, sh, sw, pt, pl, Ho, Wo, k_pad);
+    tfsc_launch(k_im2col_v8, dim3(grid), dim3(TPB), 0, s, x, y,
+                N, H, W, C, R, S, sh, sw, pt, pl, Ho, Wo, k_pad);
   } else {
     int64_t n = rows * R;
     int grid = int(ceil_div(n, (int64_t)TPB));
     if (grid > MAX_BLOCKS) grid = MAX_BLOCKS;
-    hipLaunchKernelGGL(k_im2col_row, dim3(grid), dim3(TPB), 0, s, x, y,
-                       N, H, W, C, R, S, sh, sw, pt, pl, Ho, Wo, k_pad);
+    tfsc_launch(k_im2col_row, dim3(grid), dim3(TPB), 0, s, x, y,
+                N, H, W, C, R, S, sh, sw, pt, pl, Ho, Wo, k_pad);
   }
 }
 
diff --git a/tfservingcache_amd/engine/csrc/ops/gemm.hip b/tfservingcache_amd/engine/csrc/ops/gemm.hip
--- a/tfservingcache_amd/engine/csrc/ops/gemm.hip
+++ b/tfservingcache_amd/engine/csrc/ops/gemm.hip
@@ -1,5 +1,6 @@
 #include "../common.h"
 #include "../kernels.h"
+#include "../launch.h"
 
 #include <stdexcept>
 
@@ -266,8 +267,8 @@
   dim3 block(WMW * WNW * WAVE);
   bool hb = bias != nullptr, hr = residual != nullptr;
   auto launch = [&](auto kern) {
-    hipLaunchKernelGGL(kern, grid, block, 0, s, A, B, bias, residual, C,
-                       (int)M, (int)N, (int)K, act, alpha, sA, sB, sC, ntm);
+    tfsc_launch(kern, grid, block, 0, s, A, B, bias, residual, C,
+                (int)M, (int)N, (int)K, act, alpha, sA, sB, sC, ntm);
   };
   if (hb && hr)  launch(gemm_bf16_kernel<WMW, WNW, TRANS_B, true, true>);
   else if (hb)   launch(gemm_bf16_kernel<WMW, WNW, TRANS_B, true, false>);
@@ -429,13 +430,13 @@
   int ntm = int(ceil_div(M, BM)), ntn = int(ceil_div(Kc, BN));
   dim3 grid(ntm * ntn);
   if (residual)
-    hipLaunchKernelGGL((conv_igemm_kernel<true>), grid, dim3(THREADS), 0,
-                       s, x, w, bias, residual, zeros, y, M, Kc, k_pad,
-                       act, g, ntm);
+    tfsc_launch((conv_igemm_kernel<true>), grid, dim3(THREADS), 0,
+                s, x, w, bias, residual, zeros, y, M, Kc, k_pad,
+                act, g, ntm);
   else
-    hipLaunchKernelGGL((conv_igemm_kernel<false>), grid, dim3(THREADS), 0,
-                       s, x, w, bias, nullptr, zeros, y, M, Kc, k_pad,
-                       act, g, ntm);
+    tfsc_launch((conv_igemm_kernel<false>), grid, dim3(THREADS), 0,
+                s, x, w, bias, nullptr, zeros, y, M, Kc, k_pad,
+                act, g, ntm);
 }
 
 void launch_batched_gemm(hipStream_t s, const ushort* A, const ushort* B,
diff --git a/tfservingcache_amd/engine/csrc/ops/gemm_fp8.hip b/tfservingcache_amd/engine/csrc/ops/gemm_fp8.hip
--- a/tfservingcache_amd/engine/csrc/ops/gemm_fp8.hip
+++ b/tfservingcache_amd/engine/csrc/ops/gemm_fp8.hip
@@ -1,5 +1,6 @@
 #include "../common.h"
 #include "../kernels.h"
+#include "../launch.h"
 
 #include <stdexcept>
 
@@ -288,8 +289,8 @@
   int blocks = int(ceil_div(waves_needed, (int64_t)(256 / WAVE)));
   if (blocks > 2048) blocks = 2048;
   if (blocks < 1) blocks = 1;
-  hipLaunchKernelGGL(fp8::quant_rowwise_kernel, dim3(blocks), dim3(256),
-                     0, s, x, q, scales, int(M), int(K), int(Kp));
+  tfsc_launch(fp8::quant_rowwise_kernel, dim3(blocks), dim3(256),
+              0, s, x, q, scales, int(M), int(K), int(Kp));
 }
 
 void launch_gemm_fp8(hipStream_t s, const uint8_t* A, const float* sa,
@@ -309,8 +310,8 @@
     int ntn = int(ceil_div(N, (int64_t)bn));
     dim3 grid(ntm * ntn);
     dim3 block((bm / 64) * (bn / 64) * WAVE);
-    hipLaunchKernelGGL(kern, grid, block, 0, s, A, sa, B, sb, bias,
-                       residual, C, int(M), int(N), int(K), act, ntm);
+    tfsc_launch(kern, grid, block, 0, s, A, sa, B, sb, bias,
+                residual, C, int(M), int(N), int(K), act, ntm);
   };
   if (blocks(128, 128) >= 232) {
     if (hb && hr)  go(gemm_fp8_kernel<2, 2, true, true>, 128, 128);
diff --git a/tfservingcache_amd/engine/csrc/ops/ops_memory.hip b/tfservingcache_amd/engine/csrc/ops/ops_memory.hip
--- a/tfservingcache_amd/engine/csrc/ops/ops_memory.hip
+++ b/tfservingcache_amd/engine/csrc/ops/ops_memory.hip
@@ -1,5 +1,6 @@
 #include "../common.h"
 #include "../kernels.h"
+#include "../launch.h"
 
 #include <stdexcept>
 #include <string>
@@ -103,8 +104,8 @@
 
 void launch_eltwise_unary(hipStream_t s, const ushort* x, ushort* y,
                           int64_t n, int fn) {
-  hipLaunchKernelGGL(k_unary, dim3(grid_for(n, 4)), dim3(TPB), 0, s,
-                     x, y, n, fn);
+  tfsc_launch(k_unary, dim3(grid_for(n, 4)), dim3(TPB), 0, s,
+              x, y, n, fn);
 }
 
 void launch_eltwise_binary(hipStream_t s, const ushort* a, const ushort* b,
@@ -114,11 +115,11 @@
   for (int d = 0; d < bc.ndim; ++d) {
   }
   if (bc.ndim == 1 && bc.sa[0] == 1 && bc.sb[0] == 1) {
-    hipLaunchKernelGGL(k_binary_same, dim3(grid_for(n_out, 4)), dim3(TPB),
-                       0, s, a, b, y, n_out, fn);
+    tfsc_launch(k_binary_same, dim3(grid_for(n_out, 4)), dim3(TPB),
+                0, s, a, b, y, n_out, fn);
   } else {
-    hipLaunchKernelGGL(k_binary_bcast, dim3(grid_for(n_out)), dim3(TPB),
-                       0, s, a, b, y, n_out, bc, fn);
+    tfsc_launch(k_binary_bcast, dim3(grid_for(n_out)), dim3(TPB),
+                0, s, a, b, y, n_out, bc, fn);
   }
   (void)same;
 }
@@ -148,8 +149,8 @@
                    const ushort* shift, ushort* y, int64_t rows, int64_t c,
                    int act) {
   int64_t n = rows * c;
-  hipLaunchKernelGGL(k_bn_act, dim3(grid_for(n)), dim3(TPB), 0, s,
-                     x, scale, shift, y, n, c, act);
+  tfsc_launch(k_bn_act, dim3(grid_for(n)), dim3(TPB), 0, s,
+              x, scale, shift, y, n, c, act);
 }
 
 template <typename Reduce>
@@ -242,16 +243,16 @@
     int64_t wgs = ceil_div(rows, (int64_t)(TPB / WAVE));
     int blocks = int(wgs < MAX_BLOCKS ? (wgs > 0 ? wgs : 1) : MAX_BLOCKS);
     if (cols <= 128)
-      hipLaunchKernelGGL(k_softmax_wave<2>, dim3(blocks), dim3(TPB), 0, s,
-                         x, y, rows, int(cols));
+      tfsc_launch(k_softmax_wave<2>, dim3(blocks), dim3(TPB), 0, s,
+                  x, y, rows, int(cols));
     else
-      hipLaunchKernelGGL(k_softmax_wave<8>, dim3(blocks), dim3(TPB), 0, s,
-                         x, y, rows, int(cols));
+      tfsc_launch(k_softmax_wave<8>, dim3(blocks), dim3(TPB), 0, s,
+                  x, y, rows, int(cols));
     return;
   }
   int blocks = int(rows < MAX_BLOCKS ? rows : MAX_BLOCKS);
-  hipLaunchKernelGGL(k_softmax, dim3(blocks), dim3(TPB), 0, s,
-                     x, y, rows, cols);
+  tfsc_launch(k_softmax, dim3(blocks), dim3(TPB), 0, s,
+              x, y, rows, cols);
 }
 
 __global__ void k_layernorm(const ushort* __restrict__ x,
@@ -284,8 +285,8 @@
                       const ushort* beta, ushort* y, int64_t rows,
                       int64_t cols, float eps) {
   int blocks = int(rows < MAX_BLOCKS ? rows : MAX_BLOCKS);
-  hipLaunchKernelGGL(k_layernorm, dim3(blocks), dim3(TPB), 0, s,
-                     x, gamma, beta, y, rows, cols, eps);
+  tfsc_launch(k_layernorm, dim3(blocks), dim3(TPB), 0, s,
+              x, gamma, beta, y, rows, cols, eps);
 }
 
 __global__ void k_mean_last(const ushort* __restrict__ x,
@@ -304,8 +305,8 @@
 void launch_reduce_mean_last(hipStream_t s, const ushort* x, ushort* y,
                              int64_t rows, int64_t cols) {
   int blocks = int(rows < MAX_BLOCKS ? rows : MAX_BLOCKS);
-  hipLaunchKernelGGL(k_mean_last, dim3(blocks), dim3(TPB), 0, s,
-                     x, y, rows, cols);
+  tfsc_launch(k_mean_last, dim3(blocks), dim3(TPB), 0, s,
+              x, y, rows, cols);
 }
 
 __global__ void k_mean_mid(const ushort* __restrict__ x,
@@ -325,8 +326,8 @@
 
 void launch_reduce_mean_mid(hipStream_t s, const ushort* x, ushort* y,
                             int64_t d0, int64_t d1, int64_t d2) {
-  hipLaunchKernelGGL(k_mean_mid, dim3(grid_for(d0 * d2)), dim3(TPB), 0, s,
-                     x, y, d0, d1, d2);
+  tfsc_launch(k_mean_mid, dim3(grid_for(d0 * d2)), dim3(TPB), 0, s,
+              x, y, d0, d1, d2);
 }
 
 void launch_global_mean(hipStream_t s, const ushort* x, ushort* y,
@@ -425,15 +426,15 @@
                  int sh, int sw, int pt, int pl) {
   if (C % 8 == 0) {
     int64_t n_grp = (int64_t)N * Ho * Wo * (C / 8);
-    hipLaunchKernelGGL(k_pool_v8, dim3(grid_for(n_grp)), dim3(TPB), 0, s,
-                       x, y, is_max, N, H, W, C, Ho, Wo, kh, kw, sh, sw,
-                       pt, pl);
+    tfsc_launch(k_pool_v8, dim3(grid_for(n_grp)), dim3(TPB), 0, s,
+                x, y, is_max, N, H, W, C, Ho, Wo, kh, kw, sh, sw,
+                pt, pl);
     return;
   }
   int64_t n_out = (int64_t)N * Ho * Wo * C;
-  hipLaunchKernelGGL(k_pool, dim3(grid_for(n_out)), dim3(TPB), 0, s,
-                     x, y, is_max, N, H, W, C, Ho, Wo, kh, kw, sh, sw,
-                     pt, pl);
+  tfsc_launch(k_pool, dim3(grid_for(n_out)), dim3(TPB), 0, s,
+              x, y, is_max, N, H, W, C, Ho, Wo, kh, kw, sh, sw,
+              pt, pl);
 }
 
 struct TransArgs {
@@ -494,12 +495,12 @@
   int last = ndim > 0 ? int(out_dims[ndim - 1]) : 0;
   if (ndim >= 2 && in_strides[ndim - 1] == 1 && last % 8 == 0) {
     int64_t n_grp = n_out / 8;
-    hipLaunchKernelGGL(k_transpose_v8, dim3(grid_for(n_grp)), dim3(TPB),
-                       0, s, x, y, ta, n_grp, last);
+    tfsc_launch(k_transpose_v8, dim3(grid_for(n_grp)), dim3(TPB),
+                0, s, x, y, ta, n_grp, last);
     return;
   }
-  hipLaunchKernelGGL(k_transpose, dim3(grid_for(n_out)), dim3(TPB), 0, s,
-                     x, y, ta, n_out);
+  tfsc_launch(k_transpose, dim3(grid_for(n_out)), dim3(TPB), 0, s,
+              x, y, ta, n_out);
 }
 
 __global__ void k_gather_rows(const ushort* __restrict__ table,
@@ -517,8 +518,8 @@
 
 void launch_gather_rows(hipStream_t s, const ushort* table, const int* idx,
                         ushort* y, int64_t n_idx, int64_t row_elems) {
-  hipLaunchKernelGGL(k_gather_rows, dim3(grid_for(n_idx * row_elems)),
-                     dim3(TPB), 0, s, table, idx, y, n_idx, row_elems);
+  tfsc_launch(k_gather_rows, dim3(grid_for(n_idx * row_elems)),
+              dim3(TPB), 0, s, table, idx, y, n_idx, row_elems);
 }
 
 __global__ void k_f32_to_bf16(const float* __restrict__ x,
@@ -555,14 +556,14 @@
 
 void launch_f32_to_bf16(hipStream_t s, const float* x, ushort* y,
                         int64_t n) {
-  hipLaunchKernelGGL(k_f32_to_bf16, dim3(grid_for(n, 4)), dim3(TPB), 0, s,
-                     x, y, n);
+  tfsc_launch(k_f32_to_bf16, dim3(grid_for(n, 4)), dim3(TPB), 0, s,
+              x, y, n);
 }
 
 void launch_bf16_to_f32(hipStream_t s, const ushort* x, float* y,
                         int64_t n) {
-  hipLaunchKernelGGL(k_bf16_to_f32, dim3(grid_for(n, 4)), dim3(TPB), 0, s,
-                     x, y, n);
+  tfsc_launch(k_bf16_to_f32, dim3(grid_for(n, 4)), dim3(TPB), 0, s,
+              x, y, n);
 }
 
 __global__ void k_pad_last(const ushort* __restrict__ x,
@@ -580,8 +581,8 @@
 
 void launch_pad_last(hipStream_t s, const ushort* x, ushort* y,
                      int64_t rows, int c_in, int c_out) {
-  hipLaunchKernelGGL(k_pad_last, dim3(grid_for(rows * c_out)), dim3(TPB),
-                     0, s, x, y, rows, c_in, c_out);
+  tfsc_launch(k_pad_last, dim3(grid_for(rows * c_out)), dim3(TPB),
+              0, s, x, y, rows, c_in, c_out);
 }
 
 __global__ void k_pad_nhwc(const ushort* __restrict__ x,
@@ -608,8 +609,8 @@
                      int pr) {
   int Ho = H + pt + pb, Wo = W + pl + pr;
   int64_t n_out = (int64_t)N * Ho * Wo * C;
-  hipLaunchKernelGGL(k_pad_nhwc, dim3(grid_for(n_out)), dim3(TPB), 0, s,
-                     x, y, N, H, W, C, pt, pl, Ho, Wo);
+  tfsc_launch(k_pad_nhwc, dim3(grid_for(n_out)), dim3(TPB), 0, s,
+              x, y, N, H, W, C, pt, pl, Ho, Wo);
 }
 
 TFSC_DEV float dw_act(float v, int act) {
@@ -707,14 +708,14 @@
                            int act) {
   if (C % 4 == 0) {
     int64_t total = (int64_t)N * Ho * Wo * (C / 4);
-    hipLaunchKernelGGL(k_depthwise_v4, dim3(grid_for(total)), dim3(TPB),
-                       0, s, x, w, bias, y, N, H, W, C, R, S, sh, sw,
-                       pt, pl, Ho, Wo, act);
+    tfsc_launch(k_depthwise_v4, dim3(grid_for(total)), dim3(TPB),
+                0, s, x, w, bias, y, N, H, W, C, R, S, sh, sw,
+                pt, pl, Ho, Wo, act);
   } else {
     int64_t total = (int64_t)N * Ho * Wo * C;
-    hipLaunchKernelGGL(k_depthwise_scalar, dim3(grid_for(total)),
-                       dim3(TPB), 0, s, x, w, bias, y, N, H, W, C, R, S,
-                       sh, sw, pt, pl, Ho, Wo, act);
+    tfsc_launch(k_depthwise_scalar, dim3(grid_for(total)),
+                dim3(TPB), 0, s, x, w, bias, y, N, H, W, C, R, S,
+                sh, sw, pt, pl, Ho, Wo, act);
   }
 }
 
@@ -745,8 +746,8 @@
     ta.out_dims[d] = d < ndim ? in_dims[d] : 1;
     ta.in_strides[d] = d < ndim ? out_strides[d] : 0;
   }
-  hipLaunchKernelGGL(k_scatter, dim3(grid_for(n_in)), dim3(TPB), 0, s,
-                     x, y, ta, n_in);
+  tfsc_launch(k_scatter, dim3(grid_for(n_in)), dim3(TPB), 0, s,
+              x, y, ta, n_in);
 }
 
 __global__ void k_cast_i2f(const int* __restrict__ x,
@@ -768,13 +769,13 @@
 void launch_cast(hipStream_t s, const void* x, void* y, int64_t n,
                  int mode) {
   if (mode == 0)
-    hipLaunchKernelGGL(k_cast_i2f, dim3(grid_for(n)), dim3(TPB), 0, s,
-                       reinterpret_cast<const int*>(x),
-                       reinterpret_cast<ushort*>(y), n);
+    tfsc_launch(k_cast_i2f, dim3(grid_for(n)), dim3(TPB), 0, s,
+                reinterpret_cast<const int*>(x),
+                reinterpret_cast<ushort*>(y), n);
   else
-    hipLaunchKernelGGL(k_cast_f2i, dim3(grid_for(n)), dim3(TPB), 0, s,
-                       reinterpret_cast<const ushort*>(x),
-                       reinterpret_cast<int*>(y), n);
+    tfsc_launch(k_cast_f2i, dim3(grid_for(n)), dim3(TPB), 0, s,
+                reinterpret_cast<const ushort*>(x),
+                reinterpret_cast<int*>(y), n);
 }
 
 __global__ __launch_bounds__(256)
@@ -814,8 +815,8 @@
   int blocks = int(ceil_div(waves, (int64_t)(256 / WAVE)));
   if (blocks > 2048) blocks = 2048;
   if (blocks < 1) blocks = 1;
-  hipLaunchKernelGGL(k_argmax_last, dim3(blocks), dim3(256), 0, s, x, y,
-                     rows, cols);
+  tfsc_launch(k_argmax_last, dim3(blocks), dim3(256), 0, s, x, y,
+              rows, cols);
 }
 
 struct ResizeGeom {
@@ -955,20 +956,20 @@
   if (C % 8 == 0 && aligned16(x, y)) {
     int64_t n_grp = (int64_t)N * Ho * Wo * (C / 8);
     if (mode == 1)
-      hipLaunchKernelGGL(k_resize_v8<true>, dim3(grid_for(n_grp)),
-                         dim3(TPB), 0, s, x, y, g);
+      tfsc_launch(k_resize_v8<true>, dim3(grid_for(n_grp)),
+                  dim3(TPB), 0, s, x, y, g);
     else
-      hipLaunchKernelGGL(k_resize_v8<false>, dim3(grid_for(n_grp)),
-                         dim3(TPB), 0, s, x, y, g);
+      tfsc_launch(k_resize_v8<false>, dim3(grid_for(n_grp)),
+                  dim3(TPB), 0, s, x, y, g);
     return;
   }
   int64_t n_out = (int64_t)N * Ho * Wo * C;
   if (mode == 1)
-    hipLaunchKernelGGL(k_resize<true>, dim3(grid_for(n_out)), dim3(TPB), 0,
-                       s, x, y, g);
+    tfsc_launch(k_resize<true>, dim3(grid_for(n_out)), dim3(TPB), 0,
+                s, x, y, g);
   else
-    hipLaunchKernelGGL(k_resize<false>, dim3(grid_for(n_out)), dim3(TPB), 0,
-                       s, x, y, g);
+    tfsc_launch(k_resize<false>, dim3(grid_for(n_out)), dim3(TPB), 0,
+                s, x, y, g);
 }
 
 __global__ void k_zero_insert_v8(const ushort* __restrict__ x,
@@ -1021,13 +1022,13 @@
   int Ho = int(Ho64), Wo = int(Wo64);
   if (C % 8 == 0 && aligned16(x, y)) {
     int64_t n_grp = (int64_t)N * Ho * Wo * (C / 8);
-    hipLaunchKernelGGL(k_zero_insert_v8, dim3(grid_for(n_grp)), dim3(TPB),
-                       0, s, x, y, N, h, w, C, sh, sw, Ho, Wo);
+    tfsc_launch(k_zero_insert_v8, dim3(grid_for(n_grp)), dim3(TPB),
+                0, s, x, y, N, h, w, C, sh, sw, Ho, Wo);
     return;
   }
   int64_t n_out = (int64_t)N * Ho * Wo * C;
-  hipLaunchKernelGGL(k_zero_insert, dim3(grid_for(n_out)), dim3(TPB), 0, s,
-                     x, y, N, h, w, C, sh, sw, Ho, Wo);
-}
-
-}
+  tfsc_launch(k_zero_insert, dim3(grid_for(n_out)), dim3(TPB), 0, s,
+              x, y, N, h, w, C, sh, sw, Ho, Wo);
+}
+
+}
```

Result: slower. 305.3 req/s (-2.4%).
